# grantjr1842/index-tts

Measured on AMD Instinct MI355X. Metric: synthesised audio seconds per second (IndexTTS-2 infer_v2 hot path), whole job, higher is better.
Workload: dtype f32 (greedy decode + its prefill: exact fp32 MFMA; fp32 accumulate and fp32 activations everywhere) + split-bf16 (fp32 operands as hi+lo bf16, 3 bf16 MFMAs per product) GEMMs, DiT attention and convolutions in s2mel, the latent pass and the vocoder; GPT linear weights STORED as bf16 (rounded once at

## Files before the change

index-tts_amd/csrc/gemm.h:

```cpp
#pragma once
#include "common.h"

namespace idxtts {

enum GemmAct { ACT_NONE = 0, ACT_GELU_NEW = 1, ACT_SILU = 2, ACT_SWIGLU = 3, ACT_MISH = 4, ACT_GATE = 5 ,
               ACT_GELU_ERF = 6 , ACT_RELU = 7  };

struct LinearWeights {
  const float* wp = nullptr;
  const float* bias = nullptr;
  int N = 0, K = 0;
  const void* tiles16 = nullptr;
  const void* planes16 = nullptr;
  bool mf16 = false;
};

static inline size_t linear_packed_floats(int N, int K) { return (size_t)cdiv(N, 32) * cdiv(K, 16) * 512; }

void pack_linear(float* dst, const float* w, int N, int K);

struct GemmArgs {
  const float* x = nullptr; int ldx = 0;
  float* y = nullptr; int ldy = 0;
  const void* x_planes = nullptr;
  void* y_planes = nullptr;
  const float* rope = nullptr; int rope_T = 0, rope_cols = 0;
  const float* res = nullptr; int ldr = 0;
  int M = 0;
  int act = ACT_NONE;
  float out_scale = 1.0f;
  int taps = 1, seq_len = 0, dil = 1, pad_left = 0, pad_mode = 0;
  const int* row_len = nullptr;
  int ksplit = 1;
  int bf16_products = 3;
};

int gemm_tn_forward(const LinearWeights& w, const GemmArgs& a, hipStream_t stream);
int gemm_bf16x3_forward(const LinearWeights& w, const GemmArgs& a, hipStream_t stream);
static inline bool linear_takes_planes(int N, int K) { return N >= 96 && K % 16 == 0; }
size_t linear_tiles_bytes(int N, int K);
void pack_linear_tiles(void* dst, const float* w, int N, int K);
size_t linear_planes_bytes(int N, int K);
void pack_linear_planes(void* dst, const float* w, int N, int K);

enum GemmMode { GEMM_F32 = 0, GEMM_BF16X3 = 1 };
void set_gemm_mode(int mode);
int get_gemm_mode();
void set_acoustic_bf16(int on);
int get_acoustic_bf16();
bool acoustic_bf16_active();
int gemm_forward(const LinearWeights& w, const GemmArgs& a, hipStream_t stream);
bool gemm_uses_planes(const LinearWeights& w, const GemmArgs& a);

int gemm_release_stream_scratch(hipStream_t stream);

}
```

index-tts_amd/csrc/gemm_bf16x3_v2.hip:

```cpp
#include <algorithm>
#include <cstdlib>
#include <cstring>

#include "gemm_common.h"
#include "prof.h"

namespace idxtts {

typedef __bf16 bf16x8 __attribute__((ext_vector_type(8)));
typedef __bf16 bf16x4 __attribute__((ext_vector_type(4)));

size_t linear_planes_bytes(int N, int K) { return (size_t)2 * cdiv(K, 16) * (cdiv(N, 256) * 256) * 16 * sizeof(uint16_t); }

void pack_linear_planes(void* dst, const float* w, int N, int K) {
  uint16_t* o = static_cast<uint16_t*>(dst);
  const int KC = cdiv(K, 16), NP = cdiv(N, 256) * 256;
  std::memset(o, 0, linear_planes_bytes(N, K));
  uint16_t* lo = o + (size_t)KC * NP * 16;
  for (int n = 0; n < N; ++n)
    for (int k = 0; k < K; ++k) {
      const float x = w[(size_t)n * K + k];
      const uint16_t hi = f2bf(x);
      const size_t idx = ((size_t)(k >> 4) * NP + n) * 16 + (k & 15);
      o[idx] = hi;
      lo[idx] = f2bf(x - bf2f(hi));
    }
}

__global__ __launch_bounds__(256) void split_planes_kernel(const float* __restrict__ x, int ldx, int M, int K, __bf16* __restrict__ hi,
                                                           __bf16* __restrict__ lo) {
  const int k = blockIdx.y * 64 + (threadIdx.x & 15) * 4;
#pragma unroll
  for (int i = 0; i < 4; ++i) {
    const int m = blockIdx.x * 64 + (threadIdx.x >> 4) + 16 * i;
    if (m >= M || k >= ((K + 15) & ~15)) continue;
    const f32x4 v = k < K ? *reinterpret_cast<const f32x4*>(x + (size_t)m * ldx + k) : f32x4{0.f, 0.f, 0.f, 0.f};
    bf16x4 h, l;
    split_bf16_x4(v, h, l);
    const size_t o = ((size_t)(k >> 4) * M + m) * 16 + (k & 15);
    *reinterpret_cast<bf16x4*>(hi + o) = h;
    *reinterpret_cast<bf16x4*>(lo + o) = l;
  }
}

#ifdef V2_TIMING
static unsigned long long* g_v2_stamps = nullptr;
extern "C" int idxtts_dbg_v2_stamps(void* buf) { g_v2_stamps = static_cast<unsigned long long*>(buf); return 0; }
#define V2_STAMP(k) do { if (q.stamps && tid == 64) q.stamps[(size_t)blockIdx.x * 8 + (k)] = __builtin_amdgcn_s_memtime(); } while (0)
#define V2_RSTAMP(k) do { if (q.stamps && tid == 64) q.stamps[(size_t)blockIdx.x * 8 + (k)] = __builtin_amdgcn_s_memrealtime(); } while (0)
#else
#define V2_STAMP(k)
#define V2_RSTAMP(k)
#endif

struct GemmV2P {
  GemmKP g;
  const __bf16* a_hi; const __bf16* a_lo;
  const __bf16* b_hi; const __bf16* b_lo;
  int a_rows, npad, nstages;
  int a_bytes, b_bytes;
  int a_plane, b_plane;
  int cs, nbg;
#ifdef V2_TIMING
  unsigned long long* stamps;
#endif
};

struct V2Rsrc { __amdgpu_buffer_rsrc_t a, b; };

#define V2_WAITCNT(vm) __builtin_amdgcn_s_waitcnt(((vm) & 15) | (((vm) >> 4) << 14) | 0x70)

template <bool TAPS, int EPI, int MF, int NP = 3>
__device__ __forceinline__ void gemm_v2_tile(const GemmV2P& q, const int bm, const int bn, const int tid) {
  constexpr int NSTAGE = 3;
  constexpr int WMW = 2, WNW = 2, TN = 2;
  constexpr int BM = 64 * WMW, BN = 32 * TN * WNW;
  static_assert(BM / 32 == WMW * WNW && BN / 32 == WMW * WNW, "one 32-row block of A and of B per wave and plane");
  static_assert(MF == 32 || MF == 16, "MFMA shape");
  static_assert(NP == 3 || (NP == 1 && MF == 16), "one MFMA per product exists in the 16x16x32 loop only");
  constexpr int PLANE = BM * 32;
  constexpr int STAGE_BYTES = 4 * PLANE;
  constexpr int PPW = NP == 1 ? 2 : 4;
  const GemmKP& p = q.g;
  extern __shared__ __attribute__((aligned(1024))) char smv2[];

  const int wave = __builtin_amdgcn_readfirstlane(tid >> 6), lane = tid & 63;
  const int h = lane >> 5, j = lane & 31;
  const int wm = wave >> 1, wn = wave & 1;

  const int lrow = lane >> 1;
  const int dunit = (lane & 1) ^ ((lrow >> 3) & 1);
  const int a_m = bm * BM + 32 * wave + lrow;
  const __amdgpu_buffer_rsrc_t rA = __builtin_amdgcn_make_buffer_rsrc(const_cast<__bf16*>(q.a_hi), 0, q.a_bytes, 0x00020000);
  const __amdgpu_buffer_rsrc_t rB = __builtin_amdgcn_make_buffer_rsrc(const_cast<__bf16*>(q.b_hi), 0, q.b_bytes, 0x00020000);
  const int voffB = (bn * BN + 32 * wave + lrow) * 32 + dunit * 16;
  int voffA = min(a_m, q.a_rows - 1) * 32 + dunit * 16;
  const ConvRow arow = conv_row(p, a_m);
  auto tap_voff = [&](int tap) -> int {
    const int t = conv_src_row(arow.t + tap * p.dil - p.pad_left, arow.n, p.pad_mode);
    return a_m < p.M && t >= 0 ? (arow.base + t) * 32 + dunit * 16 : (int)0x80000000;
  };
  V2_STAMP(0); V2_RSTAMP(4);
  const int ns = q.nstages;
  const int sA = q.a_rows * 32, sB = q.npad * 32;
  const int cpt = TAPS ? (p.kc >> 4) : ns;
  int ist = 0, soA = 0, soB = 0, ich = 0, itap = 0, wslot = 0, rslot = 0;
  if (TAPS) voffA = tap_voff(0);
  char* const lds_w = smv2 + wave * 1024;
  auto issue_piece = [&](int pi) {
    auto dst = (__attribute__((address_space(3))) void*)(lds_w + wslot * STAGE_BYTES + pi * PLANE);
    if (pi == 0) __builtin_amdgcn_raw_ptr_buffer_load_lds(rA, dst, 16, voffA, soA, 0, 0);
    else if (pi == 1) __builtin_amdgcn_raw_ptr_buffer_load_lds(rA, dst, 16, voffA, soA + q.a_plane, 0, 0);
    else if (pi == 2) __builtin_amdgcn_raw_ptr_buffer_load_lds(rB, dst, 16, voffB, soB, 0, 0);
    else __builtin_amdgcn_raw_ptr_buffer_load_lds(rB, dst, 16, voffB, soB + q.b_plane, 0, 0);
  };
  auto issue_a = [&]() { issue_piece(0); if (NP == 3) issue_piece(1); };
  auto issue_b = [&]() { issue_piece(2); if (NP == 3) issue_piece(3); };
  auto advance = [&]() {
    ++ist;
    wslot = wslot + 1 == NSTAGE ? 0 : wslot + 1;
    soB += sB;
    soA += sA;
    if (TAPS) {
      if (++ich == cpt) { ich = 0; soA = 0; ++itap; voffA = tap_voff(itap); }
    }
  };

  if constexpr (MF == 16) {
    const int g = lane >> 4, r16 = lane & 15;
    const int sw = ((g & 1) ^ ((r16 >> 3) & 1)) * 16;
    const int a_off = (wm * 64 + r16) * 32 + sw;
    const int b_off = 2 * PLANE + (wn * 64 + r16) * 32 + sw;
    f32x4 acc[4][4];
#pragma unroll
    for (int a = 0; a < 4; ++a)
#pragma unroll
      for (int b = 0; b < 4; ++b)
#pragma unroll
        for (int r = 0; r < 4; ++r) acc[a][b][r] = 0.0f;
    for (int s = 0; s < NSTAGE; ++s)
      if (s < ns) {
        issue_a(); issue_b();
        advance();
      }

    typedef unsigned u32x4 __attribute__((ext_vector_type(4)));
    auto pair_step = [&](const bool tail, const bool vm_one_behind, const int nreq) {
      if (vm_one_behind) V2_WAITCNT(PPW); else V2_WAITCNT(0);
      __builtin_amdgcn_s_barrier();
      __builtin_amdgcn_sched_barrier(0);
      const int second = rslot + 1 == NSTAGE ? 0 : rslot + 1;
      const char* st = smv2 + ((g >> 1) && !tail ? second : rslot) * STAGE_BYTES;
      rslot = second + 1 == NSTAGE ? 0 : second + 1;
      bf16x8 ah[4], al[4], bh[4], bl[4];
      auto rd_a = [&](int t) {
        ah[t] = *reinterpret_cast<const bf16x8*>(st + a_off + t * 512);
        if (NP == 3) al[t] = *reinterpret_cast<const bf16x8*>(st + PLANE + a_off + t * 512);
      };
      auto rd_b = [&](int t) {
        bh[t] = *reinterpret_cast<const bf16x8*>(st + b_off + t * 512);
        if (NP == 3) bl[t] = *reinterpret_cast<const bf16x8*>(st + PLANE + b_off + t * 512);
      };
      rd_a(0); rd_b(0);
      __builtin_amdgcn_sched_barrier(0);
      rd_a(1);
      __builtin_amdgcn_sched_barrier(0);
      rd_a(2);
      __builtin_amdgcn_sched_barrier(0);
      rd_a(3);
      __builtin_amdgcn_sched_barrier(0);
#pragma unroll
      for (int t = 1; t < 4; ++t) rd_b(t);
      if (tail) {
        const unsigned keep = (g >> 1) ? 0u : 0xffffffffu;
#pragma unroll
        for (int t = 0; t < 4; ++t) {
          ah[t] = (bf16x8)((u32x4)ah[t] & keep); if (NP == 3) al[t] = (bf16x8)((u32x4)al[t] & keep);
          bh[t] = (bf16x8)((u32x4)bh[t] & keep); if (NP == 3) bl[t] = (bf16x8)((u32x4)bl[t] & keep);
        }
      }
      auto prod = [&](int mt, int nt) {
        if (NP == 3) {
          acc[mt][nt] = __builtin_amdgcn_mfma_f32_16x16x32_bf16(al[mt], bh[nt], acc[mt][nt], 0, 0, 0);
          acc[mt][nt] = __builtin_amdgcn_mfma_f32_16x16x32_bf16(ah[mt], bl[nt], acc[mt][nt], 0, 0, 0);
        }
        acc[mt][nt] = __builtin_amdgcn_mfma_f32_16x16x32_bf16(ah[mt], bh[nt], acc[mt][nt], 0, 0, 0);
      };
#define V2_MFMA3(nt) _Pragma("unroll") for (int mt = 0; mt < 4; ++mt) prod(mt, nt);
#define V2_MFMA1(mt, nt) prod(mt, nt); __builtin_amdgcn_sched_barrier(0);

      __builtin_amdgcn_sched_barrier(0);
      V2_MFMA1(0, 0) V2_MFMA1(1, 0) V2_MFMA1(2, 0) V2_MFMA1(3, 0)
      V2_WAITCNT(63);
      __builtin_amdgcn_s_barrier();
      __builtin_amdgcn_sched_barrier(0);
      if (nreq >= 1) issue_a();
      __builtin_amdgcn_sched_barrier(0);
      V2_MFMA3(1)
      __builtin_amdgcn_sched_barrier(0);
      if (nreq >= 1) { issue_b(); advance(); }
      if (nreq >= 2) issue_a();
      __builtin_amdgcn_sched_barrier(0);
      V2_MFMA3(2)
      __builtin_amdgcn_sched_barrier(0);
      if (nreq >= 2) { issue_b(); advance(); }
      __builtin_amdgcn_sched_barrier(0);
      V2_MFMA3(3)
      __builtin_amdgcn_sched_barrier(0);
#undef V2_MFMA1
#undef V2_MFMA3
    };
    V2_STAMP(1);
    int done = 0;
    for (; ist + 2 <= ns && ist > done + 2; done += 2) pair_step(false, true, 2);
    for (; done + 2 <= ns; done += 2) pair_step(false, ist > done + 2, min(ns - ist, 2));
    if (done < ns) pair_step(true, false, 0);
    V2_STAMP(2);
    auto write_pass = [&](int ps, float* lds, int RS) {
#pragma unroll
      for (int nt = 0; nt < 4; ++nt)
#pragma unroll
        for (int e = 0; e < 4; ++e) lds[(4 * g + e) * RS + nt * 16 + r16] = acc[ps][nt][e];
    };
    gemm_epilogue_wave<EPI, TN, 3>(p, write_pass, reinterpret_cast<float*>(smv2), bm * BM + wm * 64, bn * BN + wn * TN * 32, wave, lane);
  } else {
    const int sw = (h ^ ((j >> 3) & 1)) * 16;
    const int a_off = (wm * 64 + j) * 32 + sw;
    const int b_offr = (wn * TN * 32 + j) * 32 + sw;

    f32x16 acc[2][TN];
#pragma unroll
    for (int a = 0; a < 2; ++a)
#pragma unroll
      for (int b = 0; b < TN; ++b)
#pragma unroll
        for (int r = 0; r < 16; ++r) acc[a][b][r] = 0.0f;

    for (int s = 0; s < NSTAGE; ++s)
      if (s < ns) {
#pragma unroll
        for (int pi = 0; pi < PPW; ++pi) issue_piece(pi);
        advance();
      }

    struct Frag { bf16x8 ah[2], al[2], bh[TN], bl[TN]; };
    auto wait_stage = [&](int s) {
      const int rem = ns - 1 - s;
      if (rem >= 1) V2_WAITCNT(PPW);
      else V2_WAITCNT(0);
      __builtin_amdgcn_s_barrier();
      __builtin_amdgcn_sched_barrier(0);
    };
    auto load_frags = [&](Frag& f) {
      const char* st = smv2 + rslot * STAGE_BYTES;
      rslot = rslot + 1 == NSTAGE ? 0 : rslot + 1;
#pragma unroll
      for (int t = 0; t < 2; ++t) {
        f.ah[t] = *reinterpret_cast<const bf16x8*>(st + a_off + t * 1024);
        f.al[t] = *reinterpret_cast<const bf16x8*>(st + PLANE + a_off + t * 1024);
      }
#pragma unroll
      for (int t = 0; t < TN; ++t) {
        f.bh[t] = *reinterpret_cast<const bf16x8*>(st + 2 * PLANE + b_offr + t * 1024);
        f.bl[t] = *reinterpret_cast<const bf16x8*>(st + 3 * PLANE + b_offr + t * 1024);
      }
    };
    auto compute = [&](const Frag& f, const bool more) {
#define V2_MFMA3(mt, nt)                                                                                         \
      acc[mt][nt] = __builtin_amdgcn_mfma_f32_32x32x16_bf16(f.al[mt], f.bh[nt], acc[mt][nt], 0, 0, 0);             \
      acc[mt][nt] = __builtin_amdgcn_mfma_f32_32x32x16_bf16(f.ah[mt], f.bl[nt], acc[mt][nt], 0, 0, 0);             \
      acc[mt][nt] = __builtin_amdgcn_mfma_f32_32x32x16_bf16(f.ah[mt], f.bh[nt], acc[mt][nt], 0, 0, 0);
      V2_MFMA3(0, 0)
      __builtin_amdgcn_sched_barrier(0);
      if (more) issue_piece(0);
      __builtin_amdgcn_sched_barrier(0);
      V2_MFMA3(0, 1)
      __builtin_amdgcn_sched_barrier(0);
      if (more) issue_piece(1);
      __builtin_amdgcn_sched_barrier(0);
      V2_MFMA3(1, 0)
      __builtin_amdgcn_sched_barrier(0);
      if (more) issue_piece(2);
      __builtin_amdgcn_sched_barrier(0);
      V2_MFMA3(1, 1)
      __builtin_amdgcn_sched_barrier(0);
      if (more) { issue_piece(3); advance(); }
      __builtin_amdgcn_sched_barrier(0);
#undef V2_MFMA3
    };

    Frag f0, f1;
    {
      const int rem = ns - 1;
      if (rem >= 2) V2_WAITCNT(2 * PPW);
      else if (rem >= 1) V2_WAITCNT(PPW);
      else V2_WAITCNT(0);
      __builtin_amdgcn_s_barrier();
      __builtin_amdgcn_sched_barrier(0);
    }
    V2_STAMP(1);
    load_frags(f0);
    int i = 0;
    for (; i + NSTAGE + 1 < ns; i += 2) {
      V2_WAITCNT((NSTAGE - 2) * PPW);
      __builtin_amdgcn_s_barrier();
      __builtin_amdgcn_sched_barrier(0);
      load_frags(f1);
      compute(f0, true);
      V2_WAITCNT((NSTAGE - 2) * PPW);
      __builtin_amdgcn_s_barrier();
      __builtin_amdgcn_sched_barrier(0);
      load_frags(f0);
      compute(f1, true);
    }
    for (; i < ns; i += 2) {
      if (i + 1 < ns) { wait_stage(i + 1); load_frags(f1); }
      else V2_WAITCNT(0);
      compute(f0, ist < ns);
      if (i + 1 < ns) {
        if (i + 2 < ns) { wait_stage(i + 2); load_frags(f0); }
        else V2_WAITCNT(0);
        compute(f1, ist < ns);
      }
    }
    V2_STAMP(2);
    auto write_pass = [&](int ps, float* lds, int RS) {
      const int mt = ps >> 1, hh = ps & 1;
#pragma unroll
      for (int nt = 0; nt < TN; ++nt)
#pragma unroll
        for (int qq = 0; qq < 2; ++qq)
#pragma unroll
          for (int e = 0; e < 4; ++e) lds[(8 * qq + 4 * h + e) * RS + nt * 32 + j] = acc[mt][nt][(2 * hh + qq) * 4 + e];
    };
    gemm_epilogue_wave<EPI, TN, 3>(p, write_pass, reinterpret_cast<float*>(smv2), bm * BM + wm * 64, bn * BN + wn * TN * 32, wave, lane);
  }
  V2_STAMP(6);
#ifdef V2_TIMING
  asm volatile("s_waitcnt vmcnt(0)" ::: "memory");
#endif
  V2_STAMP(3); V2_RSTAMP(5);
}

template <bool TAPS, int EPI, int MF, int NP = 3>
__global__ __launch_bounds__(256, 3) void gemm_bf16x3_v2_kernel(const GemmV2P q) {
  int bn, bm;
  if (!gemm_tile_walk(q.g, blockIdx.x, bm, bn, q.cs, q.nbg)) return;
  gemm_v2_tile<TAPS, EPI, MF, NP>(q, bm, bn, threadIdx.x);
}

StreamScratch g_plane_scratch(8);

int gemm_bf16x3_v2_forward(GemmKP p, const LinearWeights& w, const GemmArgs& a, hipStream_t stream, double flops, double bytes) {
  IDX_CHECK(w.K % 16 == 0 && (a.taps <= 1 || (w.K / a.taps) % 16 == 0), "v2 needs K % 16 == 0");
  const int xk = a.taps > 1 ? w.K / a.taps : w.K;
  const size_t plane = (size_t)(xk / 16) * a.M * 16 * sizeof(__bf16);
  void* scratch = nullptr;
  if (!a.x_planes && g_plane_scratch.acquire(stream, 2 * plane, &scratch)) return 1;
  const __bf16* hi = static_cast<const __bf16*>(a.x_planes ? a.x_planes : scratch);
  const __bf16* lo = hi + plane / sizeof(__bf16);
  if (!a.x_planes) {
    static const int cat_split = prof_register("split_planes_kernel");
    ProfScope prof(cat_split, stream, 0.0, 8.0 * a.M * (double)xk);
    hipLaunchKernelGGL(split_planes_kernel, dim3(cdiv(a.M, 64), cdiv(xk, 64)), dim3(256), 0, stream, a.x, a.ldx, a.M, xk, const_cast<__bf16*>(hi), const_cast<__bf16*>(lo));
    IDX_LAUNCH_CHECK();
  }
  GemmV2P q;
  q.g = p;
  if (a.y_planes) {
    const int n_out = (a.act == ACT_SWIGLU || a.act == ACT_GATE) ? w.N / 2 : w.N;
    IDX_CHECK(n_out % 16 == 0 && (a.ldy & 3) == 0, "output planes need N_out % 16 == 0");
    q.g.y_hi = static_cast<__bf16*>(a.y_planes);
    q.g.y_lo = q.g.y_hi + plane_elems(a.M, n_out);
  }
  if (a.rope) {
    IDX_CHECK(a.rope_T > 0 && a.rope_cols % 64 == 0 && a.act == ACT_NONE && (a.ldy & 3) == 0, "fused rotary arguments");
    q.g.rope = a.rope; q.g.rope_T = a.rope_T; q.g.rope_cols = a.rope_cols;
  }
  const int BMh = 128, BNh = 128;
  q.g.mtiles = cdiv(a.M, BMh);
  q.g.mt8 = cdiv(q.g.mtiles, 8);
  q.g.nblocks = cdiv(w.N, BNh);
  q.a_hi = hi; q.a_lo = lo; q.a_rows = a.M;
  q.npad = cdiv(w.N, 256) * 256;
  q.b_hi = static_cast<const __bf16*>(w.planes16);
  q.b_lo = q.b_hi + (size_t)(w.K / 16) * q.npad * 16;
  q.nstages = w.K / 16;
#ifdef V2_TIMING
  q.stamps = g_v2_stamps;
#endif
  const size_t b_plane = (size_t)(w.K / 16) * q.npad * 32;
  IDX_CHECK(2 * plane < (1ull << 31) && 2 * b_plane < (1ull << 31), "operand planes beyond the 2 GiB a buffer offset addresses");
  q.a_plane = (int)plane; q.a_bytes = (int)(2 * plane);
  q.b_plane = (int)b_plane; q.b_bytes = (int)(2 * b_plane);
  q.cs = 1;
  static const double cs_bytes = [] { const char* e = getenv("IDXTTS_GEMM_CS_BYTES"); return e ? atof(e) : 3.2e6; }();
  if (!q.g.n_fast && (double)w.N * w.K * 4.0 <= 8.0 * cs_bytes && a.M > w.N) q.g.n_fast = 1;
  if (q.g.n_fast) {
    while (q.cs < 8 && (double)w.N * w.K * 4.0 / q.cs > cs_bytes && q.g.nblocks >= 2 * q.cs) q.cs *= 2;
  }
  q.nbg = cdiv(q.g.nblocks, q.cs);
  const int64_t grid = q.g.n_fast ? (int64_t)8 * q.nbg * cdiv(q.g.mtiles, 8 / q.cs) : (int64_t)8 * q.g.nblocks * q.g.mt8;
  IDX_CHECK(grid < (1ll << 31), "grid size");
  static const int cat = prof_register("gemm_bf16x3_v2_kernel");
  ProfScope prof(cat, stream, flops, bytes);
  const int lds = 3 * (4 * 128 * 32);
  const bool paired = a.act == ACT_SWIGLU || a.act == ACT_GATE;
  IDX_CHECK(!(a.rope && (a.res || paired)), "the rotary epilogue takes no residual and no paired activation");
  IDX_CHECK(!a.row_len || a.seq_len >= 16, "row masks need seq_len >= 16");
  const int epi = a.rope ? EPI_ROPE : paired ? EPI_PAIRED : a.act != ACT_NONE ? EPI_ACT : EPI_PLAIN;
  typedef void (*KernelFn)(const GemmV2P);
#define V2_ROW(T, F, P) gemm_bf16x3_v2_kernel<T, EPI_PLAIN, F, P>, gemm_bf16x3_v2_kernel<T, EPI_ROPE, F, P>, gemm_bf16x3_v2_kernel<T, EPI_PAIRED, F, P>, gemm_bf16x3_v2_kernel<T, EPI_ACT, F, P>
  static const KernelFn kernels[3][2][4] = {{{V2_ROW(false, 32, 3)}, {V2_ROW(true, 32, 3)}}, {{V2_ROW(false, 16, 3)}, {V2_ROW(true, 16, 3)}},
                                            {{V2_ROW(false, 16, 1)}, {V2_ROW(true, 16, 1)}}};
  static DynLdsLimit lds_limit;
  IDX_HIP(lds_limit.set(lds, V2_ROW(false, 32, 3), V2_ROW(true, 32, 3), V2_ROW(false, 16, 3), V2_ROW(true, 16, 3), V2_ROW(false, 16, 1), V2_ROW(true, 16, 1)));
  IDX_CHECK(a.bf16_products == 3 || (a.bf16_products == 1 && w.mf16), "one MFMA per product needs weights of the 16x16x32 loop");
  int mf16 = w.mf16 ? 1 : 0;
#ifdef V2_EXP_SHAPE
  if (const char* e = getenv("IDXTTS_EXP_V2_SHAPE")) mf16 = atoi(e) == 16;
#endif
  const KernelFn kernel = kernels[a.bf16_products == 1 ? 2 : mf16][a.taps > 1 ? 1 : 0][epi];
#undef V2_ROW
  hipLaunchKernelGGL(kernel, dim3((unsigned)grid), dim3(256), lds, stream, q);
  IDX_LAUNCH_CHECK();
  return 0;
}

}
```

index-tts_amd/csrc/model_util.h:

```cpp
#pragma once
#include <map>
#include <string>
#include <vector>

#include "ctx.h"
#include "gemm.h"

namespace idxtts {

int need(std::map<std::string, HostTensor>& t, const std::string& key, std::vector<int64_t> shape, HostTensor** out);
int up(DeviceArena& arena, const std::vector<float>& v, const float** out);
int tensor_from(std::map<std::string, HostTensor>& t, DeviceArena& arena, const std::string& key, std::vector<int64_t> shape, const float** out);
int vec_from(std::map<std::string, HostTensor>& t, DeviceArena& arena, const std::string& key, int n, const float** out);
int ln_from(std::map<std::string, HostTensor>& t, DeviceArena& arena, const std::string& prefix, int n, const float** g, const float** b);

enum Wp16Policy {
  WP16_ALWAYS,
  WP16_DMA_SHAPES,
  WP16_ALWAYS_MF16,
  WP16_NONE,
};
enum WeightLayout { W_NK , W_KN  };
struct LinearOpts {
  Wp16Policy wp16;
  WeightLayout layout = W_NK;
  int Kpad = 0;
  bool split_bf16_below_256_rows = false;
};
int make_linear(DeviceArena& arena, const float* w, const float* bias, int N, int K, const LinearOpts& o, LinearWeights* out);
int linear_from(std::map<std::string, HostTensor>& t, DeviceArena& arena, const std::string& prefix, int N, int K, bool bias, Wp16Policy wp16,
                LinearWeights* out, std::vector<int64_t> wshape = {});

struct Carver {
  char* base; size_t off = 0;
  explicit Carver(void* b) : base(static_cast<char*>(b)) {}
  template <typename T> T* take(size_t n) {
    off = (off + 255) & ~(size_t)255;
    T* p = base ? reinterpret_cast<T*>(base + off) : nullptr;
    off += n * sizeof(T);
    return p;
  }
};

int lin(const LinearWeights& w, const float* x, int ldx, float* y, int ldy, int M, hipStream_t st, int act = ACT_NONE,
        const float* res = nullptr, int ldr = 0);
int lin_exact(const LinearWeights& w, const float* x, int ldx, float* y, int ldy, int M, hipStream_t st, int act = ACT_NONE,
              const float* res = nullptr, int ldr = 0);
int layer_norm(const float* x, float* y, const float* g, const float* b, int M, int d, hipStream_t st);

}
```

index-tts_amd/csrc/model_util.hip:

```cpp
#include "model_util.h"

#include <cstring>

#include "norm.h"

namespace idxtts {

int need(std::map<std::string, HostTensor>& t, const std::string& key, std::vector<int64_t> shape, HostTensor** out) {
  auto it = t.find(key);
  if (it == t.end()) IDX_FAIL("missing tensor '" + key + "'");
  if (it->second.shape != shape) {
    std::string s = "tensor '" + key + "' has shape [";
    for (auto d : it->second.shape) s += std::to_string(d) + ",";
    s += "] expected [";
    for (auto d : shape) s += std::to_string(d) + ",";
    IDX_FAIL(s + "]");
  }
  *out = &it->second;
  return 0;
}

int up(DeviceArena& arena, const std::vector<float>& v, const float** out) {
  float* d = nullptr;
  if (arena.upload(v.data(), v.size(), &d)) return 1;
  *out = d;
  return 0;
}

int tensor_from(std::map<std::string, HostTensor>& t, DeviceArena& arena, const std::string& key, std::vector<int64_t> shape, const float** out) {
  HostTensor* h = nullptr;
  if (need(t, key, shape, &h)) return 1;
  return up(arena, h->data, out);
}

int vec_from(std::map<std::string, HostTensor>& t, DeviceArena& arena, const std::string& key, int n, const float** out) {
  return tensor_from(t, arena, key, {n}, out);
}

int ln_from(std::map<std::string, HostTensor>& t, DeviceArena& arena, const std::string& prefix, int n, const float** g, const float** b) {
  return vec_from(t, arena, prefix + ".weight", n, g) || vec_from(t, arena, prefix + ".bias", n, b);
}

int make_linear(DeviceArena& arena, const float* w, const float* bias, int N, int K, const LinearOpts& o, LinearWeights* out) {
  const int Kpad = o.Kpad ? o.Kpad : K;
  IDX_CHECK(Kpad >= K, "Kpad < K");
  std::vector<float> rows;
  if (o.layout == W_KN || Kpad != K) {
    rows.assign((size_t)N * Kpad, 0.0f);
    for (int n = 0; n < N; ++n)
      for (int k = 0; k < K; ++k) rows[(size_t)n * Kpad + k] = o.layout == W_KN ? w[(size_t)k * N + n] : w[(size_t)n * K + k];
    w = rows.data();
  }
  std::vector<float> packed(linear_packed_floats(N, Kpad));
  pack_linear(packed.data(), w, N, Kpad);
  if (up(arena, packed, &out->wp)) return 1;
  out->N = N; out->K = Kpad;
  out->mf16 = o.wp16 == WP16_ALWAYS_MF16;
  auto pack16 = [&](size_t bytes, void (*pack)(void*, const float*, int, int), const void** dst) {
    std::vector<float> p16((bytes + 3) / 4);
    pack(p16.data(), w, N, Kpad);
    const float* d16 = nullptr;
    if (up(arena, p16, &d16)) return 1;
    *dst = d16;
    return 0;
  };
  const bool planes = o.wp16 != WP16_NONE && linear_takes_planes(N, Kpad);
  const bool tiles = o.wp16 != WP16_NONE && (o.split_bf16_below_256_rows || (o.wp16 != WP16_DMA_SHAPES && !planes));
  if (planes && pack16(linear_planes_bytes(N, Kpad), pack_linear_planes, &out->planes16)) return 1;
  if (tiles && pack16(linear_tiles_bytes(N, Kpad), pack_linear_tiles, &out->tiles16)) return 1;
  if (bias && up(arena, std::vector<float>(bias, bias + N), &out->bias)) return 1;
  return 0;
}

int linear_from(std::map<std::string, HostTensor>& t, DeviceArena& arena, const std::string& prefix, int N, int K, bool bias, Wp16Policy wp16,
                LinearWeights* out, std::vector<int64_t> wshape) {
  HostTensor *w = nullptr, *b = nullptr;
  if (wshape.empty()) wshape = {N, K};
  if (need(t, prefix + ".weight", wshape, &w)) return 1;
  if (bias && need(t, prefix + ".bias", {N}, &b)) return 1;
  return make_linear(arena, w->data.data(), b ? b->data.data() : nullptr, N, K, {wp16, W_NK, (K + 3) & ~3}, out);
}

static GemmArgs lin_args(const float* x, int ldx, float* y, int ldy, int M, int act, const float* res, int ldr) {
  GemmArgs g;
  g.x = x; g.ldx = ldx; g.y = y; g.ldy = ldy; g.M = M; g.act = act; g.res = res; g.ldr = ldr;
  return g;
}

int lin(const LinearWeights& w, const float* x, int ldx, float* y, int ldy, int M, hipStream_t st, int act, const float* res, int ldr) {
  const GemmArgs g = lin_args(x, ldx, y, ldy, M, act, res, ldr);
  if (act == ACT_GELU_ERF || act == ACT_RELU) return gemm_tn_forward(w, g, st);
  return gemm_forward(w, g, st);
}

int lin_exact(const LinearWeights& w, const float* x, int ldx, float* y, int ldy, int M, hipStream_t st, int act, const float* res, int ldr) {
  return gemm_tn_forward(w, lin_args(x, ldx, y, ldy, M, act, res, ldr), st);
}

int layer_norm(const float* x, float* y, const float* g, const float* b, int M, int d, hipStream_t st) {
  RowsNormArgs n;
  n.x_in = x; n.ld_in = d; n.y = y; n.ld_y = d; n.M = M; n.d = d; n.mode = NORM_LN; n.eps = 1e-5f; n.g1 = g; n.b1 = b;
  return rows_norm_forward(n, st);
}

}
```

index-tts_amd/csrc/s2mel.hip:

```cpp
#include <cmath>
#include <cstring>

#include <map>
#include <mutex>
#include <utility>

#include "model_util.h"
#include "s2mel.h"
#include "s2mel_buffers.h"

namespace idxtts {

S2MelModel::S2MelModel(const idxtts_s2mel_config& c) : cfg(c) {}

bool S2MelModel::accepts(const std::string& name) const {
  static const char* prefixes[] = {"cfm.estimator.", "length_regulator.", "gpt_layer.", "semantic_codec.", "rope_cache"};
  for (const char* p : prefixes)
    if (name.rfind(p, 0) == 0) return true;
  return false;
}

namespace {

std::vector<float> col_slice(const std::vector<float>& w, int N, int K, int k0, int k1) {
  std::vector<float> o((size_t)N * (k1 - k0));
  for (int n = 0; n < N; ++n) std::memcpy(&o[(size_t)n * (k1 - k0)], &w[(size_t)n * K + k0], (k1 - k0) * sizeof(float));
  return o;
}

std::vector<float> pair_pack(const float* a, const float* b, int H, int K) {
  std::vector<float> o((size_t)2 * H * K);
  for (int blk = 0; blk < H / 32; ++blk) {
    std::memcpy(&o[(size_t)(blk * 64) * K], a + (size_t)blk * 32 * K, (size_t)32 * K * sizeof(float));
    std::memcpy(&o[(size_t)(blk * 64 + 32) * K], b + (size_t)blk * 32 * K, (size_t)32 * K * sizeof(float));
  }
  return o;
}

std::vector<float> conv_to_rows(const std::vector<float>& w, int Cout, int Cin, int k) {
  std::vector<float> o((size_t)Cout * Cin * k);
  for (int co = 0; co < Cout; ++co)
    for (int ci = 0; ci < Cin; ++ci)
      for (int kk = 0; kk < k; ++kk) o[((size_t)co * k + kk) * Cin + ci] = w[((size_t)co * Cin + ci) * k + kk];
  return o;
}

}

int S2MelModel::finalize(std::map<std::string, HostTensor>& t, DeviceArena& arena) {
  const int D = cfg.hidden_dim, C = cfg.in_channels, Wh = cfg.wn_hidden, depth = cfg.depth;
  IDX_CHECK(D == cfg.num_heads * 64, "head_dim must be 64");
  IDX_CHECK(Wh == D, "the reference's FinalLayer requires wavenet.hidden_dim == DiT.hidden_dim");
  IDX_CHECK((D & 31) == 0 && (Wh & 31) == 0 && (cfg.lr_channels & 31) == 0, "channel counts must be multiples of 32");
  {
    const int nh = (int)(2 * (4 * D) / 3);
    ffn = (nh % 256 == 0) ? nh : nh + 256 - (nh % 256);
  }
  const std::string e = "cfm.estimator";
  auto lin_from = [&](const std::string& key, int N, int K, bool bias, LinearWeights* out) { return linear_from(t, arena, key, N, K, bias, WP16_ALWAYS_MF16, out); };
  auto mk_lin = [&](const float* w, const float* bias, int N, int K, LinearWeights* out) { return make_linear(arena, w, bias, N, K, {WP16_ALWAYS_MF16}, out); };
  blocks.resize(depth);
  std::vector<float> mod_w, mod_b;
  auto append_mod = [&](const std::string& name) -> int {
    HostTensor *w = nullptr, *b = nullptr;
    if (need(t, name + ".project_layer.weight", {2 * D, D}, &w) || need(t, name + ".project_layer.bias", {2 * D}, &b)) return 1;
    mod_w.insert(mod_w.end(), w->data.begin(), w->data.end());
    mod_b.insert(mod_b.end(), b->data.begin(), b->data.end());
    return 0;
  };
  for (int i = 0; i < depth; ++i) {
    DiTBlock& B = blocks[i];
    const std::string p = e + ".transformer.layers." + std::to_string(i);
    if (lin_from(p + ".attention.wqkv", 3 * D, D, false, &B.wqkv)) return 1;
    if (lin_from(p + ".attention.wo", D, D, false, &B.wo)) return 1;
    HostTensor *w1 = nullptr, *w3 = nullptr;
    if (need(t, p + ".feed_forward.w1.weight", {ffn, D}, &w1) || need(t, p + ".feed_forward.w3.weight", {ffn, D}, &w3)) return 1;
    if (mk_lin(pair_pack(w1->data.data(), w3->data.data(), ffn, D).data(), nullptr, 2 * ffn, D, &B.w13)) return 1;
    if (lin_from(p + ".feed_forward.w2", D, ffn, false, &B.w2)) return 1;
    HostTensor *g = nullptr;
    if (need(t, p + ".attention_norm.norm.weight", {D}, &g) || up(arena, g->data, &B.attn_g)) return 1;
    if (need(t, p + ".ffn_norm.norm.weight", {D}, &g) || up(arena, g->data, &B.ffn_g)) return 1;
    if (append_mod(p + ".attention_norm") || append_mod(p + ".ffn_norm")) return 1;
    if (i > depth / 2) {
      HostTensor *sw = nullptr, *sb = nullptr;
      if (need(t, p + ".skip_in_linear.weight", {D, 2 * D}, &sw) || need(t, p + ".skip_in_linear.bias", {D}, &sb)) return 1;
      if (mk_lin(col_slice(sw->data, D, 2 * D, 0, D).data(), sb->data.data(), D, D, &B.skip_a)) return 1;
      if (mk_lin(col_slice(sw->data, D, 2 * D, D, 2 * D).data(), nullptr, D, D, &B.skip_b)) return 1;
    }
  }
  {
    HostTensor* g = nullptr;
    if (need(t, e + ".transformer.norm.norm.weight", {D}, &g) || up(arena, g->data, &final_g)) return 1;
    if (append_mod(e + ".transformer.norm")) return 1;
    if (mk_lin(mod_w.data(), mod_b.data(), (2 * depth + 1) * 2 * D, D, &mod_all)) return 1;
  }
  const int Win = 2 * C + D + cfg.style_dim;
  if (lin_from(e + ".cond_projection", D, cfg.content_dim, true, &cond_proj)) return 1;
  if (lin_from(e + ".cond_x_merge_linear", D, Win, true, &merge)) return 1;
  if (lin_from(e + ".t_embedder.mlp.0", D, 256, true, &temb0) || lin_from(e + ".t_embedder.mlp.2", D, D, true, &temb2)) return 1;
  if (lin_from(e + ".t_embedder2.mlp.0", Wh, 256, true, &t2emb0) || lin_from(e + ".t_embedder2.mlp.2", Wh, Wh, true, &t2emb2)) return 1;
  {
    HostTensor *sw = nullptr, *sb = nullptr;
    if (need(t, e + ".skip_linear.weight", {D, D + C}, &sw) || need(t, e + ".skip_linear.bias", {D}, &sb)) return 1;
    if (mk_lin(col_slice(sw->data, D, D + C, 0, D).data(), sb->data.data(), D, D, &skiplin_a)) return 1;
    if (mk_lin(col_slice(sw->data, D, D + C, D, D + C).data(), nullptr, D, C, &skiplin_b)) return 1;
  }
  if (lin_from(e + ".conv1", Wh, D, true, &conv1)) return 1;
  if (lin_from(e + ".res_projection", Wh, D, true, &res_proj)) return 1;
  if (lin_from(e + ".final_layer.linear", Wh, Wh, true, &final_lin)) return 1;
  if (lin_from(e + ".final_layer.adaLN_modulation.1", 2 * Wh, Wh, true, &final_mod)) return 1;
  {
    HostTensor *w = nullptr, *b = nullptr;
    if (need(t, e + ".conv2.weight", {C, Wh, 1}, &w) || need(t, e + ".conv2.bias", {C}, &b)) return 1;
    if (mk_lin(w->data.data(), b->data.data(), C, Wh, &conv2)) return 1;
  }
  const int L = cfg.wn_layers, k = cfg.wn_kernel;
  wn.resize(L);
  {
    HostTensor *cw = nullptr, *cb = nullptr;
    if (need(t, e + ".wavenet.cond_layer.conv.conv.weight", {2 * Wh * L, Wh, 1}, &cw) ||
        need(t, e + ".wavenet.cond_layer.conv.conv.bias", {2 * Wh * L}, &cb)) return 1;
    std::vector<float> cw_perm, cb_perm;
    for (int l = 0; l < L; ++l) {
      WNLayer& W = wn[l];
      const std::string p = e + ".wavenet.in_layers." + std::to_string(l) + ".conv.conv";
      HostTensor *iw = nullptr, *ib = nullptr;
      if (need(t, p + ".weight", {2 * Wh, Wh, k}, &iw) || need(t, p + ".bias", {2 * Wh}, &ib)) return 1;
      const std::vector<float> rows = conv_to_rows(iw->data, 2 * Wh, Wh, k);
      if (mk_lin(pair_pack(rows.data(), rows.data() + (size_t)Wh * k * Wh, Wh, k * Wh).data(), nullptr, 2 * Wh, k * Wh, &W.in_gate)) return 1;
      const float* cwl = cw->data.data() + (size_t)l * 2 * Wh * Wh;
      const std::vector<float> cwp = pair_pack(cwl, cwl + (size_t)Wh * Wh, Wh, Wh);
      cw_perm.insert(cw_perm.end(), cwp.begin(), cwp.end());
      std::vector<float> bsum(2 * Wh);
      for (int c = 0; c < 2 * Wh; ++c) bsum[c] = cb->data[(size_t)l * 2 * Wh + c] + ib->data[c];
      const std::vector<float> bp = pair_pack(bsum.data(), bsum.data() + Wh, Wh, 1);
      cb_perm.insert(cb_perm.end(), bp.begin(), bp.end());
      const std::string r = e + ".wavenet.res_skip_layers." + std::to_string(l) + ".conv.conv";
      const int rc = l < L - 1 ? 2 * Wh : Wh;
      HostTensor *rw = nullptr, *rb = nullptr;
      if (need(t, r + ".weight", {rc, Wh, 1}, &rw) || need(t, r + ".bias", {rc}, &rb)) return 1;
      if (l < L - 1) {
        std::vector<float> w_res(rw->data.begin(), rw->data.begin() + (size_t)Wh * Wh), b_res(rb->data.begin(), rb->data.begin() + Wh);
        std::vector<float> w_skip(rw->data.begin() + (size_t)Wh * Wh, rw->data.end()), b_skip(rb->data.begin() + Wh, rb->data.end());
        if (mk_lin(w_res.data(), b_res.data(), Wh, Wh, &W.res) || mk_lin(w_skip.data(), b_skip.data(), Wh, Wh, &W.skip)) return 1;
      } else {
        W.has_res = false;
        if (mk_lin(rw->data.data(), rb->data.data(), Wh, Wh, &W.skip)) return 1;
      }
    }
    if (mk_lin(cw_perm.data(), cb_perm.data(), 2 * Wh * L, Wh, &wn_cond)) return 1;
  }
  const int LC = cfg.lr_channels;
  if (lin_from("length_regulator.content_in_proj", LC, cfg.lr_in_channels, true, &lr_in)) return 1;
  lr_conv.resize(cfg.lr_num_convs);
  lr_gn_g.resize(cfg.lr_num_convs);
  lr_gn_b.resize(cfg.lr_num_convs);
  for (int n = 0; n < cfg.lr_num_convs; ++n) {
    HostTensor *w = nullptr, *b = nullptr, *g = nullptr, *bb = nullptr;
    const std::string p = "length_regulator.model." + std::to_string(3 * n);
    if (need(t, p + ".weight", {LC, LC, 3}, &w) || need(t, p + ".bias", {LC}, &b)) return 1;
    if (mk_lin(conv_to_rows(w->data, LC, LC, 3).data(), b->data.data(), LC, 3 * LC, &lr_conv[n])) return 1;
    const std::string q = "length_regulator.model." + std::to_string(3 * n + 1);
    if (need(t, q + ".weight", {LC}, &g) || need(t, q + ".bias", {LC}, &bb)) return 1;
    if (up(arena, g->data, &lr_gn_g[n]) || up(arena, bb->data, &lr_gn_b[n])) return 1;
  }
  {
    HostTensor *w = nullptr, *b = nullptr;
    const std::string p = "length_regulator.model." + std::to_string(3 * cfg.lr_num_convs);
    if (need(t, p + ".weight", {LC, LC, 1}, &w) || need(t, p + ".bias", {LC}, &b)) return 1;
    if (mk_lin(w->data.data(), b->data.data(), LC, LC, &lr_out)) return 1;
  }
  {
    const int dims[4] = {cfg.gpt_dim, cfg.gpt_layer_dims[0], cfg.gpt_layer_dims[1], cfg.gpt_layer_dims[2]};
    for (int n = 0; n < 3; ++n)
      if (lin_from("gpt_layer." + std::to_string(n), dims[n + 1], dims[n], true, &gl[n])) return 1;
    IDX_CHECK(dims[3] == cfg.codec_hidden && cfg.codec_hidden == cfg.lr_in_channels, "gpt_layer / codec / length-regulator widths");
  }
  {
    HostTensor *cb = nullptr, *ow = nullptr, *ob = nullptr;
    const std::string q = "semantic_codec.quantizer.quantizers.0";
    if (need(t, q + ".codebook.weight", {cfg.codebook_size, cfg.codebook_dim}, &cb) ||
        need(t, q + ".out_project.weight", {cfg.codec_hidden, cfg.codebook_dim, 1}, &ow) ||
        need(t, q + ".out_project.bias", {cfg.codec_hidden}, &ob)) return 1;
    std::vector<float> table((size_t)cfg.codebook_size * cfg.codec_hidden);
    for (int v = 0; v < cfg.codebook_size; ++v)
      for (int h = 0; h < cfg.codec_hidden; ++h) {
        float acc = 0.0f;
        for (int c = 0; c < cfg.codebook_dim; ++c) acc = std::fmaf(cb->data[(size_t)v * cfg.codebook_dim + c], ow->data[(size_t)h * cfg.codebook_dim + c], acc);
        table[(size_t)v * cfg.codec_hidden + h] = acc + ob->data[h];
      }
    if (up(arena, table, &vq_table)) return 1;
  }
  {
    auto it = t.find("rope_cache");
    if (it == t.end()) IDX_FAIL("missing tensor 'rope_cache' ([T][32][2] cos/sin table, precompute_freqs_cis)");
    IDX_CHECK(it->second.shape.size() == 3 && it->second.shape[1] == 32 && it->second.shape[2] == 2, "rope_cache must be [T][32][2]");
    rope_len = (int)it->second.shape[0];
    if (up(arena, it->second.data, &rope)) return 1;
  }
  return 0;
}

size_t S2MelModel::cfm_workspace_bytes(int B, int T, int n_steps) const { return carve_cfm(cfg, ffn, nullptr, B, T, n_steps).bytes; }

struct Src { const float* f; const void* p; Src(const float* rows, const void* planes = nullptr) : f(planes ? nullptr : rows), p(planes) {} };
struct Dst { float* f; void* p; Dst(float* rows, void* planes = nullptr) : f(rows), p(planes) {} };

static GemmArgs gemm_args(Src x, int ldx, Dst y, int ldy, int M, int act = ACT_NONE, const float* res = nullptr, int ldr = 0) {
  GemmArgs a;
  a.x = x.f; a.x_planes = x.p; a.ldx = ldx; a.y = y.f; a.y_planes = y.p; a.ldy = ldy; a.M = M; a.act = act; a.res = res; a.ldr = ldr;
  return a;
}
static int gemm(const LinearWeights& w, Src x, int ldx, Dst y, int ldy, int M, hipStream_t st, int act = ACT_NONE,
                const float* res = nullptr, int ldr = 0) {
  return gemm_forward(w, gemm_args(x, ldx, y, ldy, M, act, res, ldr), st);
}

struct RowSet {
  const CfmBuffers* w = nullptr;
  int nseq = 0, seq = 0, rows = 0;
  const int* lens = nullptr;
  bool planes = false;
  bool planes_wn = false;

  Src hn_in() const { return in(w->hn, w->hn_p, planes); }                  Dst hn_out() const { return instead(w->hn, w->hn_p, planes); }
  Src att_in() const { return in(w->att, w->att_p, planes); }               Dst att_out() const { return instead(w->att, w->att_p, planes); }
  Src ff_in() const { return in(w->ff, w->ff_p, planes); }                  Dst ff_out() const { return instead(w->ff, w->ff_p, planes); }
  Src acts_in() const { return in(w->wn_acts, w->acts_p, planes); }         Dst acts_out() const { return instead(w->wn_acts, w->acts_p, planes); }
  Src skip_in(int i) const { return in(w->skips[i], w->skips_p[i], planes); }   Dst skip_out(int i) const { return beside(w->skips[i], w->skips_p[i], planes); }
  Src xres_in() const { return in(w->xres, w->xres_p, planes_wn); }         Dst xres_out() const { return beside(w->xres, w->xres_p, planes_wn); }
  Src wnx_in() const { return in(w->wn_x, w->wnx_p, planes_wn); }           Dst wnx_out() const { return beside(w->wn_x, w->wnx_p, planes_wn); }
  Src h_in(const float* h) const { return in(h, w->h_p, planes); }          Dst h_out(float* h, bool reread) const { return beside(h, w->h_p, planes && reread); }

 private:
  static Src in(const float* f, const void* p, bool on) { return on ? Src(f, p) : Src(f); }
  static Dst instead(float* f, void* p, bool on) { return on ? Dst(nullptr, p) : Dst(f); }
  static Dst beside(float* f, void* p, bool on) { return on ? Dst(f, p) : Dst(f); }
};

static RowSet row_set(const S2MelModel& m, const CfmBuffers& w, int nseq, int seq, const int* lens, const RowSet* within) {
  RowSet r;
  r.w = &w; r.nseq = nseq; r.seq = seq; r.rows = nseq * seq; r.lens = lens;
  const DiTBlock& b0 = m.blocks[0];
  const WNLayer& wn0 = m.wn[0];
  GemmArgs pr;
  pr.M = r.rows;
  r.planes = within ? within->planes : gemm_uses_planes(b0.wqkv, pr);
  for (const LinearWeights* lw : {&b0.wo, &b0.w13, &b0.w2, &m.skiplin_a, &m.final_lin, &wn0.skip}) r.planes = r.planes && gemm_uses_planes(*lw, pr);
  r.planes_wn = r.planes && (!within || within->planes_wn);
  for (const LinearWeights* lw : {&m.skiplin_b, &m.conv1, &m.res_proj, &wn0.res}) r.planes_wn = r.planes_wn && gemm_uses_planes(*lw, pr);
  pr.taps = m.cfg.wn_kernel; pr.seq_len = seq;
  r.planes_wn = r.planes_wn && gemm_uses_planes(wn0.in_gate, pr);
  return r;
}

static int ada_norm(const S2MelModel& m, const float* x, const float* g, const float* mod, const RowSet& r, hipStream_t st) {
  const int D = m.cfg.hidden_dim;
  const Dst hn = r.hn_out();
  RowsNormArgs n;
  n.x_in = x; n.ld_in = D; n.y = hn.f; n.y_planes = hn.p; n.ld_y = D; n.M = r.rows; n.d = D;
  n.mode = NORM_ADA_RMS; n.eps = m.cfg.norm_eps; n.g1 = g;
  n.mod_a = mod; n.mod_b = mod + D; n.ld_mod = 0; n.rows_per_batch = 0;
  return rows_norm_forward(n, st);
}

static int attention(const S2MelModel& m, const RowSet& all, bool qkv_planes, int q0, int Sq, Dst o, hipStream_t st) {
  const int D = m.cfg.hidden_dim, T = all.seq;
  const float* qkv = all.w->qkv;
  if (qkv_planes) {
    AttnPlanesArgs ap;
    ap.planes = qkv; ap.Mrows = all.rows; ap.ncols = 3 * D; ap.q_col = 0; ap.k_col = D; ap.v_col = 2 * D; ap.T = T; ap.q_row0 = q0; ap.Sq = Sq;
    ap.B = all.nseq; ap.H = m.cfg.num_heads; ap.kend = all.lens; ap.scale = 0.125f;
    ap.o = o.f; ap.o_planes = o.p; ap.o_bs = (long)Sq * D; ap.o_ts = D;
    ap.split_bf16 = acoustic_bf16_active() ? 2 : 1;
    return flash_attn_planes_forward(ap, st);
  }
  AttnArgs a;
  a.q = qkv + (size_t)q0 * 3 * D; a.k = qkv + D; a.v = qkv + 2 * D; a.o = o.f; a.o_planes = o.p;
  a.q_bs = a.k_bs = a.v_bs = (long)T * 3 * D; a.o_bs = (long)Sq * D; a.q_ts = a.k_ts = a.v_ts = 3 * D; a.o_ts = D;
  a.B = all.nseq; a.H = m.cfg.num_heads; a.Sq = Sq; a.Sk = T; a.causal = 0; a.kend = all.lens; a.scale = 0.125f;
  a.split_bf16 = get_gemm_mode() == GEMM_BF16X3 ? (acoustic_bf16_active() ? 2 : 1) : 0;
  return flash_attn_forward(a, st);
}

static int dit_block(S2MelModel& m, int i, const float* mods, const float* h, const RowSet& all, const RowSet& post, float* res, Dst out,
                     hipEvent_t lag_event, hipStream_t st) {
  const auto& c = m.cfg;
  const CfmBuffers& w = *all.w;
  const DiTBlock& B = m.blocks[i];
  const int D = c.hidden_dim, T = all.seq, q0 = T - post.seq;
  if (ada_norm(m, h, B.attn_g, mods + (size_t)(2 * i) * 2 * D, all, st)) return 1;
  bool qkv_planes = false;
  {
    GemmArgs g = gemm_args(all.hn_in(), D, w.qkv, 3 * D, all.rows);
    const bool fuse_rope = gemm_uses_planes(B.wqkv, g);
    qkv_planes = fuse_rope && D == 64 * c.num_heads;
    if (fuse_rope) { g.rope = m.rope; g.rope_T = T; g.rope_cols = 2 * D; }
    if (qkv_planes) { g.y = nullptr; g.y_planes = w.qkv; }
    if (gemm_forward(B.wqkv, g, st)) return 1;
    if (!fuse_rope && rotary_qk(w.qkv, all.rows, c.num_heads, T, m.rope, st)) return 1;
  }
  if (attention(m, all, qkv_planes, q0, post.seq, post.att_out(), st)) return 1;
  if (lag_event) IDX_HIP(hipEventRecord(lag_event, st));
  if (res != h && gather_tail_rows(res, D, h, D, D, all.nseq, T, q0, st)) return 1;
  if (gemm(B.wo, post.att_in(), D, w.hmid, D, post.rows, st, ACT_NONE, res, D)) return 1;
  if (ada_norm(m, w.hmid, B.ffn_g, mods + (size_t)(2 * i + 1) * 2 * D, post, st)) return 1;
  if (gemm(B.w13, post.hn_in(), D, post.ff_out(), m.ffn, post.rows, st, ACT_SWIGLU)) return 1;
  return gemm(B.w2, post.ff_in(), m.ffn, out, D, post.rows, st, ACT_NONE, w.hmid, D);
}

static int dit_eval(S2MelModel& m, CfmBuffers& w, int N2, int T, int step, hipStream_t st, hipEvent_t lag_event) {
  const auto& c = m.cfg;
  const int D = c.hidden_dim, C = c.in_channels, Wh = c.wn_hidden, depth = c.depth, half = depth / 2;
  const int Win = 2 * C + D + c.style_dim;
  const float* mods = w.mods + (size_t)step * (2 * depth + 1) * 2 * D;
  const int t0 = w.tail_t0;
  const RowSet all = row_set(m, w, N2, T, w.lens2, nullptr);
  const RowSet tail = t0 > 0 ? row_set(m, w, N2, T - t0, w.lens2t, &all) : all;
  if (lag_event && depth < 2) IDX_HIP(hipEventRecord(lag_event, st));
  if (gemm(m.merge, w.x_in, Win, w.ha, D, all.rows, st)) return 1;
  float* h = w.ha;
  int pushed = 0;
  for (int i = 0; i < depth; ++i) {
    if (i > half) {
      DiTBlock& B = m.blocks[i];
      --pushed;
      if (gemm(B.skip_a, all.h_in(h), D, w.hmid, D, all.rows, st)) return 1;
      float* dst = (h == w.ha) ? w.hb : w.ha;
      if (gemm(B.skip_b, all.skip_in(pushed), D, dst, D, all.rows, st, ACT_NONE, w.hmid, D)) return 1;
      h = dst;
    }
    const Dst out = i < half ? all.skip_out(pushed) : all.h_out((h == w.ha) ? w.hb : w.ha, i + 1 < depth && i + 1 > half);
    const bool cut = i == depth - 1 && t0 > 0;
    if (dit_block(m, i, mods, h, all, cut ? tail : all, cut ? w.xres : h, out, i == 0 && !cut ? lag_event : nullptr, st)) return 1;
    if (i < half) ++pushed;
    h = out.f;
  }
  const int Mt = tail.rows, Tt = tail.seq;
  const float* xin_t = w.x_in;
  int ld_xin = Win;
  if (t0 > 0) {
    if (gather_tail_rows(w.qkv, C, w.x_in, Win, C, N2, T, t0, st)) return 1;
    xin_t = w.qkv; ld_xin = C;
  }
  if (ada_norm(m, h, m.final_g, mods + (size_t)(2 * depth) * 2 * D, tail, st)) return 1;
  if (gemm(m.skiplin_a, tail.hn_in(), D, w.hmid, D, Mt, st)) return 1;
  if (gemm(m.skiplin_b, xin_t, ld_xin, tail.xres_out(), D, Mt, st, ACT_NONE, w.hmid, D)) return 1;
  if (gemm(m.conv1, tail.xres_in(), D, tail.wnx_out(), Wh, Mt, st)) return 1;
  const int L = c.wn_layers, k = c.wn_kernel;
  for (int l = 0; l < L; ++l) {
    WNLayer& W = m.wn[l];
    int dil = 1;
    for (int q = 0; q < l; ++q) dil *= c.wn_dilation_rate;
    LinearWeights in = W.in_gate;
    in.bias = w.wnb + ((size_t)step * L + l) * 2 * Wh;
    GemmArgs g = gemm_args(tail.wnx_in(), Wh, tail.acts_out(), Wh, Mt, ACT_GATE);
    g.taps = k; g.seq_len = Tt; g.dil = dil; g.pad_left = (k - 1) / 2 * dil; g.pad_mode = 1; g.row_len = tail.lens;
    if (gemm_forward(in, g, st)) return 1;
    if (W.has_res) {
      GemmArgs r = gemm_args(tail.acts_in(), Wh, tail.wnx_out(), Wh, Mt, ACT_NONE, w.wn_x, Wh);
      r.seq_len = Tt; r.row_len = tail.lens;
      if (gemm_forward(W.res, r, st)) return 1;
    }
    GemmArgs sk = gemm_args(tail.acts_in(), Wh, w.wn_out, Wh, Mt);
    if (l > 0) { sk.res = w.wn_out; sk.ldr = Wh; }
    if (l == L - 1) { sk.seq_len = Tt; sk.row_len = tail.lens; }
    if (gemm_forward(W.skip, sk, st)) return 1;
  }
  if (gemm(m.res_proj, tail.xres_in(), D, w.hmid, Wh, Mt, st, ACT_NONE, w.wn_out, Wh)) return 1;
  {
    const Dst hn = tail.hn_out();
    RowsNormArgs n;
    n.x_in = w.hmid; n.ld_in = Wh; n.y = hn.f; n.y_planes = hn.p; n.ld_y = Wh; n.M = Mt; n.d = Wh; n.mode = NORM_MOD_LN; n.eps = 1e-6f;
    n.mod_a = w.fmod + (size_t)step * 2 * Wh; n.mod_b = n.mod_a + Wh; n.ld_mod = 0; n.rows_per_batch = 0;
    if (rows_norm_forward(n, st)) return 1;
  }
  if (gemm(m.final_lin, tail.hn_in(), Wh, w.att, Wh, Mt, st)) return 1;
  return gemm(m.conv2, w.att, Wh, w.vout, C, Mt, st);
}

struct HalfStreams { hipStream_t side = nullptr; hipEvent_t fork = nullptr, lag = nullptr, join = nullptr; };
static std::map<std::pair<int, hipStream_t>, HalfStreams> g_half_streams;
static std::mutex g_half_mu;
static int g_s2mel_overlap = 0;
void set_s2mel_overlap(int on) { g_s2mel_overlap = on ? 1 : 0; }
int get_s2mel_overlap() { return g_s2mel_overlap; }

static int half_streams_for(hipStream_t st, HalfStreams* out) {
  int dev = 0;
  IDX_HIP(hipGetDevice(&dev));
  std::lock_guard<std::mutex> lk(g_half_mu);
  HalfStreams& hs = g_half_streams[std::make_pair(dev, st)];
  if (!hs.side) {
    int prio = 0;
    if (st) IDX_HIP(hipStreamGetPriority(st, &prio));
    IDX_HIP(hipStreamCreateWithPriority(&hs.side, hipStreamNonBlocking, prio));
    IDX_HIP(hipEventCreateWithFlags(&hs.fork, hipEventDisableTiming));
    IDX_HIP(hipEventCreateWithFlags(&hs.lag, hipEventDisableTiming));
    IDX_HIP(hipEventCreateWithFlags(&hs.join, hipEventDisableTiming));
  }
  *out = hs;
  return 0;
}

int s2mel_release_stream(hipStream_t st) {
  int dev = 0;
  IDX_HIP(hipGetDevice(&dev));
  HalfStreams hs;
  {
    std::lock_guard<std::mutex> lk(g_half_mu);
    auto it = g_half_streams.find(std::make_pair(dev, st));
    if (it == g_half_streams.end()) return 0;
    hs = it->second;
    g_half_streams.erase(it);
  }
  if (hs.side) { (void)hipStreamSynchronize(hs.side); (void)hipStreamDestroy(hs.side); }
  if (hs.fork) (void)hipEventDestroy(hs.fork);
  if (hs.lag) (void)hipEventDestroy(hs.lag);
  if (hs.join) (void)hipEventDestroy(hs.join);
  return 0;
}

static bool halves_on_two_streams(hipStream_t st) {
  hipStreamCaptureStatus cap = hipStreamCaptureStatusNone;
  (void)hipStreamIsCapturing(st, &cap);
  return g_s2mel_overlap && !prof_enabled() && cap == hipStreamCaptureStatusNone;
}

static int dit_eval_halves(S2MelModel& m, CfmBuffers& w, int B, int T, int step, bool two_streams, hipStream_t st) {
  if (!two_streams) return dit_eval(m, w, 2 * B, T, step, st, nullptr);
  CfmBuffers v0 = half_view(m.cfg, m.ffn, w, 0, B, T);
  CfmBuffers v1 = half_view(m.cfg, m.ffn, w, 1, B, T);
  HalfStreams hs;
  if (half_streams_for(st, &hs)) return 1;
  IDX_HIP(hipEventRecord(hs.fork, st));
  IDX_HIP(hipStreamWaitEvent(hs.side, hs.fork, 0));
  if (dit_eval(m, v0, B, T, step, st, hs.lag)) return 1;
  IDX_HIP(hipStreamWaitEvent(hs.side, hs.lag, 0));
  if (dit_eval(m, v1, B, T, step, hs.side, nullptr)) return 1;
  IDX_HIP(hipEventRecord(hs.join, hs.side));
  IDX_HIP(hipStreamWaitEvent(st, hs.join, 0));
  return 0;
}

int S2MelModel::cfm(const float* mu, const int* x_lens_host, const float* prompt, const int* prompt_lens_host, int Tp_max,
                    const float* style, const float* z, const float* t_emb, const float* dt_host, int n_steps, float cfg_rate,
                    float* out, int B, int T, void* ws, size_t ws_bytes, hipStream_t st) {
  IDX_CHECK(mu && x_lens_host && prompt && prompt_lens_host && style && z && t_emb && dt_host && out, "null pointer");
  IDX_CHECK(B > 0 && T > 0 && n_steps > 0 && Tp_max > 0, "shape");
  IDX_CHECK(cfg_rate > 0.0f, "the stacked-CFG path needs inference_cfg_rate > 0 (reference default 0.7)");
  IDX_CHECK(T <= rope_len, "sequence longer than the rope cache");
  IDX_CHECK(ws && ws_bytes >= cfm_workspace_bytes(B, T, n_steps), "workspace too small");
  CfmBuffers w = carve_cfm(cfg, ffn, ws, B, T, n_steps);
  if (cfm_solve(w, mu, x_lens_host, prompt, prompt_lens_host, Tp_max, style, z, t_emb, dt_host, n_steps, cfg_rate, B, T, st)) return 1;
  IDX_HIP(hipMemcpyAsync(out, w.xstate, (size_t)B * cfg.in_channels * T * sizeof(float), hipMemcpyDeviceToDevice, st));
  return 0;
}

static int upload_lens(const S2MelModel& m, CfmBuffers& w, const int* x_lens_host, const int* prompt_lens_host, int Tp_max, int B, int T,
                       bool solver, hipStream_t st) {
  const auto& c = m.cfg;
  std::vector<int> lens2(2 * B), plen(B), lens2t(2 * B);
  for (int b = 0; b < B; ++b) {
    const int pmax = std::min(Tp_max, solver ? x_lens_host[b] : T);
    IDX_CHECK(x_lens_host[b] > 0 && x_lens_host[b] <= T && prompt_lens_host[b] >= 0 && prompt_lens_host[b] <= pmax, "lengths");
    lens2[b] = lens2[B + b] = x_lens_host[b];
    plen[b] = prompt_lens_host[b];
  }
  IDX_HIP(hipMemcpyAsync(w.lens2, lens2.data(), 2 * B * sizeof(int), hipMemcpyHostToDevice, st));
  if (solver) {
    int halo = 0, dil = 1, pmin = plen[0];
    for (int l = 0; l < c.wn_layers; ++l) { halo += (c.wn_kernel - 1) / 2 * dil; dil *= c.wn_dilation_rate; }
    for (int b = 0; b < B; ++b) pmin = std::min(pmin, plen[b]);
    w.tail_t0 = pmin - halo >= 64 ? pmin - halo : 0;
    for (int i = 0; i < 2 * B; ++i) lens2t[i] = lens2[i] - w.tail_t0;
    IDX_HIP(hipMemcpyAsync(w.lens2t, lens2t.data(), 2 * B * sizeof(int), hipMemcpyHostToDevice, st));
  }
  IDX_HIP(hipMemcpyAsync(w.plen, plen.data(), B * sizeof(int), hipMemcpyHostToDevice, st));
  IDX_HIP(hipStreamSynchronize(st));
  return 0;
}

static int step_constants(const S2MelModel& m, const CfmBuffers& w, const float* t_emb, int n_steps, hipStream_t st) {
  const int D = m.cfg.hidden_dim, Wh = m.cfg.wn_hidden;
  if (gemm(m.temb0, t_emb, 256, w.tmp_steps, D, n_steps, st, ACT_SILU) || gemm(m.temb2, w.tmp_steps, D, w.t1, D, n_steps, st)) return 1;
  if (gemm(m.mod_all, w.t1, D, w.mods, (2 * m.cfg.depth + 1) * 2 * D, n_steps, st)) return 1;
  if (silu_rows(w.t1s, w.t1, (size_t)n_steps * D, st) || gemm(m.final_mod, w.t1s, Wh, w.fmod, 2 * Wh, n_steps, st)) return 1;
  if (gemm(m.t2emb0, t_emb, 256, w.tmp_steps, Wh, n_steps, st, ACT_SILU) || gemm(m.t2emb2, w.tmp_steps, Wh, w.t2, Wh, n_steps, st)) return 1;
  return gemm(m.wn_cond, w.t2, Wh, w.wnb, m.cfg.wn_layers * 2 * Wh, n_steps, st);
}

static CfmPackArgs pack_args(const S2MelModel& m, const CfmBuffers& w, const float* prompt, const float* style, int B, int T, int Tp_max) {
  const auto& c = m.cfg;
  CfmPackArgs pk;
  pk.x_in = w.x_in; pk.ld = 2 * c.in_channels + c.hidden_dim + c.style_dim; pk.x = w.xstate; pk.prompt = prompt; pk.prompt_len = w.plen;
  pk.cond = w.condp; pk.cond_null = m.cond_proj.bias; pk.style = style;
  pk.B = B; pk.T = T; pk.C = c.in_channels; pk.D = c.hidden_dim; pk.S = c.style_dim; pk.Tp_max = Tp_max;
  return pk;
}

int S2MelModel::cfm_solve(CfmBuffers& w, const float* mu, const int* x_lens_host, const float* prompt, const int* prompt_lens_host,
                          int Tp_max, const float* style, const float* z, const float* t_emb, const float* dt_host, int n_steps,
                          float cfg_rate, int B, int T, hipStream_t st) {
  const int D = cfg.hidden_dim, C = cfg.in_channels;
  if (upload_lens(*this, w, x_lens_host, prompt_lens_host, Tp_max, B, T, true, st)) return 1;
  if (step_constants(*this, w, t_emb, n_steps, st)) return 1;
  if (gemm(cond_proj, mu, cfg.content_dim, w.condp, D, B * T, st)) return 1;
  if (cfm_init_state(w.xstate, z, w.plen, B, C, T, st)) return 1;
  const bool two_streams = halves_on_two_streams(st);
  for (int s = 0; s < n_steps; ++s) {
    CfmPackArgs pk = pack_args(*this, w, prompt, style, B, T, Tp_max);
    pk.x_only = s > 0;
    if (cfm_pack(pk, st)) return 1;
    if (dit_eval_halves(*this, w, B, T, s, two_streams, st)) return 1;
    CfmEulerArgs eu;
    eu.x = w.xstate; eu.v = w.vout; eu.v_null = two_streams ? w.vout + (size_t)B * T * C : nullptr; eu.ldv = C; eu.prompt_len = w.plen; eu.B = B; eu.T = T; eu.C = C; eu.dt = dt_host[s]; eu.cfg_rate = cfg_rate;
    eu.v_t0 = w.tail_t0; eu.v_T = T - w.tail_t0;
    if (cfm_euler(eu, st)) return 1;
  }
  return 0;
}

struct CfmRowsBuffers { float *mu, *prompt; const float **pcond, **ref_mel; int* gen_len; size_t bytes; };

static CfmRowsBuffers carve_cfm_rows(const S2MelModel& m, void* ws, size_t base, int B, int T, int Tp_max) {
  const auto& c = m.cfg;
  CfmRowsBuffers b;
  Carver k(ws ? static_cast<char*>(ws) + base : nullptr);
  b.mu = k.take<float>((size_t)B * T * c.content_dim);
  b.prompt = k.take<float>((size_t)B * c.in_channels * Tp_max);
  b.pcond = k.take<const float*>(B);
  b.ref_mel = k.take<const float*>(B);
  b.gen_len = k.take<int>(B);
  b.bytes = base + ((k.off + 255) & ~(size_t)255);
  return b;
}

size_t S2MelModel::cfm_rows_workspace_bytes(int B, int T, int Tp_max, int n_steps) const {
  return carve_cfm_rows(*this, nullptr, cfm_workspace_bytes(B, T, n_steps), B, T, Tp_max).bytes;
}

int S2MelModel::cfm_rows(const float* gen_cond, const int* target_lens_host, int Tg_max, const float* const* prompt_cond_host,
                         const float* const* ref_mel_host, const int* prompt_lens_host, const float* style, const float* z,
                         const float* t_emb, const float* dt_host, int n_steps, float cfg_rate, float* out, int B, int T, void* ws,
                         size_t ws_bytes, hipStream_t st) {
  IDX_CHECK(gen_cond && target_lens_host && prompt_cond_host && ref_mel_host && prompt_lens_host && style && z && t_emb && dt_host && out,
            "null pointer");
  IDX_CHECK(B > 0 && T > 0 && Tg_max > 0 && n_steps > 0, "shape");
  IDX_CHECK(cfg_rate > 0.0f, "the stacked-CFG path needs inference_cfg_rate > 0 (reference default 0.7)");
  IDX_CHECK(T <= rope_len, "sequence longer than the rope cache");
  IDX_CHECK(cfg.content_dim % 4 == 0 && ((uintptr_t)gen_cond & 15) == 0, "gen_cond must be 16-byte aligned (content_dim % 4 == 0)");
  std::vector<int> xl(B), tg(B);
  int Tp_max = 0, T_need = 0;
  for (int b = 0; b < B; ++b) {
    const int Tp = prompt_lens_host[b], Tg = target_lens_host[b];
    IDX_CHECK(Tp > 0 && Tg > 0 && Tg <= Tg_max, "prompt_lens / target_lens out of range");
    IDX_CHECK(prompt_cond_host[b] && ref_mel_host[b], "null prompt table entry");
    IDX_CHECK(((uintptr_t)prompt_cond_host[b] & 15) == 0, "prompt_condition rows must be 16-byte aligned");
    xl[b] = Tp + Tg;
    tg[b] = Tg;
    Tp_max = std::max(Tp_max, Tp);
    T_need = std::max(T_need, Tp + Tg);
  }
  IDX_CHECK(T == T_need, "T must be max_b(prompt_lens[b] + target_lens[b])");
  IDX_CHECK(ws && ws_bytes >= cfm_rows_workspace_bytes(B, T, Tp_max, n_steps), "workspace too small");
  CfmBuffers w = carve_cfm(cfg, ffn, ws, B, T, n_steps);
  CfmRowsBuffers r = carve_cfm_rows(*this, ws, w.bytes, B, T, Tp_max);
  IDX_HIP(hipMemcpyAsync(r.pcond, prompt_cond_host, B * sizeof(float*), hipMemcpyHostToDevice, st));
  IDX_HIP(hipMemcpyAsync(r.ref_mel, ref_mel_host, B * sizeof(float*), hipMemcpyHostToDevice, st));
  IDX_HIP(hipMemcpyAsync(r.gen_len, tg.data(), B * sizeof(int), hipMemcpyHostToDevice, st));
  IDX_HIP(hipMemcpyAsync(w.plen, prompt_lens_host, B * sizeof(int), hipMemcpyHostToDevice, st));
  CfmRowsPackArgs pk;
  pk.mu = r.mu; pk.prompt = r.prompt; pk.pcond = r.pcond; pk.ref_mel = r.ref_mel; pk.gen = gen_cond; pk.prompt_len = w.plen;
  pk.gen_len = r.gen_len; pk.B = B; pk.T = T; pk.Dc = cfg.content_dim; pk.C = cfg.in_channels; pk.Tp_max = Tp_max; pk.Tg_max = Tg_max;
  if (cfm_rows_pack(pk, st)) return 1;
  if (cfm_solve(w, r.mu, xl.data(), r.prompt, prompt_lens_host, Tp_max, style, z, t_emb, dt_host, n_steps, cfg_rate, B, T, st)) return 1;
  return cfm_rows_emit(out, w.xstate, w.plen, r.gen_len, B, cfg.in_channels, T, Tg_max, st);
}

int S2MelModel::estimator(const float* x, const float* prompt, const int* prompt_lens_host, int Tp_max, const int* x_lens_host,
                          const float* t_emb, const float* style, const float* mu, float* out_tm, int B, int T, void* ws, size_t ws_bytes,
                          hipStream_t st) {
  IDX_CHECK(x && prompt && prompt_lens_host && x_lens_host && t_emb && style && mu && out_tm, "null pointer");
  IDX_CHECK(B > 0 && T > 0 && Tp_max > 0 && T <= rope_len, "shape");
  IDX_CHECK(ws && ws_bytes >= cfm_workspace_bytes(B, T, 1), "workspace too small");
  const int C = cfg.in_channels;
  CfmBuffers w = carve_cfm(cfg, ffn, ws, B, T, 1);
  if (upload_lens(*this, w, x_lens_host, prompt_lens_host, Tp_max, B, T, false, st)) return 1;
  if (step_constants(*this, w, t_emb, 1, st)) return 1;
  if (gemm(cond_proj, mu, cfg.content_dim, w.condp, cfg.hidden_dim, B * T, st)) return 1;
  IDX_HIP(hipMemcpyAsync(w.xstate, x, (size_t)B * C * T * sizeof(float), hipMemcpyDeviceToDevice, st));
  if (cfm_pack(pack_args(*this, w, prompt, style, B, T, Tp_max), st)) return 1;
  {
    CfmBuffers v0 = half_view(cfg, ffn, w, 0, B, T);
    if (dit_eval(*this, v0, B, T, 0, st, nullptr)) return 1;
  }
  IDX_HIP(hipMemcpyAsync(out_tm, w.vout, (size_t)B * T * C * sizeof(float), hipMemcpyDeviceToDevice, st));
  return 0;
}


static CondBuffers carve_cond(const S2MelModel& m, void* ws, int B, int M, int Tg) {
  const auto& c = m.cfg;
  CondBuffers b;
  Carver k(ws);
  const size_t rows = (size_t)B * std::max(M, Tg);
  const int wide = std::max(std::max(c.codec_hidden, c.lr_channels), std::max(c.gpt_layer_dims[0], c.gpt_layer_dims[1]));
  b.a = k.take<float>(rows * wide);
  b.b = k.take<float>(rows * wide);
  b.s = k.take<float>(rows * wide);
  b.stats = k.take<float>(2 * B);
  b.idx_code = k.take<int>((size_t)B * M);
  b.idx_row = k.take<int>((size_t)B * M);
  b.idx_interp = k.take<int>((size_t)B * Tg);
  b.tlen = k.take<int>(B);
  b.bytes = (k.off + 255) & ~(size_t)255;
  return b;
}

size_t S2MelModel::cond_workspace_bytes(int B, int M, int Tg) const { return carve_cond(*this, nullptr, B, M, Tg).bytes; }

static void nearest_rows(int* idx, int row0, int mb, int tb) {
  const float scale = (float)mb / (float)tb;
  for (int j = 0; j < tb; ++j) idx[j] = row0 + std::min((int)std::floor((float)j * scale), mb - 1);
}

int S2MelModel::prepare_cond(const float* latent, const long long* codes, const int* code_lens_host, const int* target_lens_host,
                             int B, int M, int Tg, float* cond_out, void* ws, size_t ws_bytes, hipStream_t st) {
  IDX_CHECK(latent && codes && code_lens_host && target_lens_host && cond_out, "null pointer");
  IDX_CHECK(B > 0 && M > 0 && Tg > 0, "shape");
  IDX_CHECK(ws && ws_bytes >= cond_workspace_bytes(B, M, Tg), "workspace too small");
  const int Hc = cfg.codec_hidden;
  CondBuffers w = carve_cond(*this, ws, B, M, Tg);
  std::vector<long long> hc((size_t)B * M);
  IDX_HIP(hipMemcpyAsync(hc.data(), codes, hc.size() * sizeof(long long), hipMemcpyDeviceToHost, st));
  IDX_HIP(hipStreamSynchronize(st));
  std::vector<int> ic((size_t)B * M), ir((size_t)B * M), ii((size_t)B * Tg, -1), tl(B);
  for (int b = 0; b < B; ++b) {
    const int mb = code_lens_host[b], tb = target_lens_host[b];
    IDX_CHECK(mb > 0 && mb <= M && tb > 0 && tb <= Tg, "code_lens / target_lens out of range");
    tl[b] = tb;
    for (int i = 0; i < M; ++i) {
      const long long cde = hc[(size_t)b * M + i];
      IDX_CHECK(i >= mb || (cde >= 0 && cde < cfg.codebook_size), "semantic code out of the codebook");
      ic[(size_t)b * M + i] = i < mb ? (int)cde : -1;
      ir[(size_t)b * M + i] = i < mb ? b * M + i : -1;
    }
    nearest_rows(&ii[(size_t)b * Tg], b * M, mb, tb);
  }
  IDX_HIP(hipMemcpyAsync(w.idx_code, ic.data(), ic.size() * sizeof(int), hipMemcpyHostToDevice, st));
  IDX_HIP(hipMemcpyAsync(w.idx_row, ir.data(), ir.size() * sizeof(int), hipMemcpyHostToDevice, st));
  IDX_HIP(hipMemcpyAsync(w.idx_interp, ii.data(), ii.size() * sizeof(int), hipMemcpyHostToDevice, st));
  IDX_HIP(hipMemcpyAsync(w.tlen, tl.data(), B * sizeof(int), hipMemcpyHostToDevice, st));
  IDX_HIP(hipStreamSynchronize(st));
  const int rowsM = B * M;
  if (gemm(gl[0], latent, cfg.gpt_dim, w.a, gl[0].N, rowsM, st) || gemm(gl[1], w.a, gl[0].N, w.b, gl[1].N, rowsM, st) ||
      gemm(gl[2], w.b, gl[1].N, w.a, Hc, rowsM, st)) return 1;
  GatherArgs ga;
  ga.out = w.s; ga.ld_out = Hc; ga.d = Hc;
  ga.table[0] = vq_table; ga.idx[0] = w.idx_code;
  ga.table[1] = w.a; ga.idx[1] = w.idx_row;
  if (gather_sum_rows(ga, rowsM, st)) return 1;
  return regulate_rows(w.s, w, B, M, Tg, cond_out, st);
}

int S2MelModel::regulate_rows(const float* s_rows, const CondBuffers& w, int B, int M, int Tg, float* cond_out, hipStream_t st) {
  const int Hc = cfg.codec_hidden, LC = cfg.lr_channels;
  const int rowsM = B * M, rowsT = B * Tg;
  if (gemm(lr_in, s_rows, Hc, w.a, LC, rowsM, st)) return 1;
  GatherArgs gi;
  gi.out = w.b; gi.ld_out = LC; gi.d = LC; gi.table[0] = w.a; gi.idx[0] = w.idx_interp;
  if (gather_sum_rows(gi, rowsT, st)) return 1;
  float* cur = w.b;
  float* other = w.a;
  for (int n = 0; n < cfg.lr_num_convs; ++n) {
    GemmArgs g;
    g.x = cur; g.ldx = LC; g.y = other; g.ldy = LC; g.M = rowsT; g.taps = 3; g.seq_len = Tg; g.dil = 1; g.pad_left = 1; g.pad_mode = 0;
    if (gemm_forward(lr_conv[n], g, st)) return 1;
    if (groupnorm1_mish(cur, other, lr_gn_g[n], lr_gn_b[n], w.tlen, B, Tg, LC, 1e-5f, w.stats, st)) return 1;
  }
  GemmArgs o;
  o.x = cur; o.ldx = LC; o.y = cond_out; o.ldy = LC; o.M = rowsT; o.seq_len = Tg; o.row_len = w.tlen;
  return gemm_forward(lr_out, o, st);
}

int S2MelModel::regulate(const float* S, const int* in_lens_host, const int* target_lens_host, int B, int M, int Tg, float* cond_out,
                         void* ws, size_t ws_bytes, hipStream_t st) {
  IDX_CHECK(S && in_lens_host && target_lens_host && cond_out, "null pointer");
  IDX_CHECK(B > 0 && M > 0 && Tg > 0, "shape");
  IDX_CHECK(ws && ws_bytes >= cond_workspace_bytes(B, M, Tg), "workspace too small");
  CondBuffers w = carve_cond(*this, ws, B, M, Tg);
  std::vector<int> ii((size_t)B * Tg, -1), tl(B);
  for (int b = 0; b < B; ++b) {
    const int mb = in_lens_host[b], tb = target_lens_host[b];
    IDX_CHECK(mb > 0 && mb <= M && tb > 0 && tb <= Tg, "in_lens / target_lens out of range");
    tl[b] = tb;
    nearest_rows(&ii[(size_t)b * Tg], b * M, mb, tb);
  }
  IDX_HIP(hipMemcpyAsync(w.idx_interp, ii.data(), ii.size() * sizeof(int), hipMemcpyHostToDevice, st));
  IDX_HIP(hipMemcpyAsync(w.tlen, tl.data(), B * sizeof(int), hipMemcpyHostToDevice, st));
  IDX_HIP(hipStreamSynchronize(st));
  return regulate_rows(S, w, B, M, Tg, cond_out, st);
}

}
```

index-tts_amd/csrc/s2mel_buffers.h:

```cpp
#pragma once
#include <algorithm>
#include <vector>

#include "../../include/idxtts.h"
#include "model_util.h"

namespace idxtts {

struct CfmBuffers {
  float *x_in, *ha, *hb, *hmid, *hn, *qkv, *att, *ff, *xres, *wn_x, *wn_acts, *wn_out, *vout, *condp, *xstate;
  void *hn_p, *att_p, *ff_p, *acts_p;
  void *h_p, *wnx_p, *xres_p;
  std::vector<void*> skips_p;
  std::vector<float*> skips;
  float *t1, *t1s, *mods, *fmod, *t2, *wnb, *tmp_steps;
  int *lens2, *plen, *lens2t;
  int tail_t0 = 0;
  size_t bytes;
};

enum CfmKind {
  CFM_ROWS,
  CFM_PLANES,
  CFM_STEPS,
  CFM_INTS,
};
constexpr bool CFM_HALVED = true, CFM_SHARED = false;

inline size_t cfm_block_elems(int B, int T, int n_steps, CfmKind kind, size_t cols) {
  return cols * (kind == CFM_STEPS ? (size_t)n_steps : kind == CFM_INTS ? (size_t)B : (size_t)B * T);
}

template <typename F> void cfm_buffer_table(CfmBuffers& b, const idxtts_s2mel_config& c, int ffn, F&& f) {
  const int D = c.hidden_dim, C = c.in_channels, Wh = c.wn_hidden;
  const CfmKind R = CFM_ROWS, P = CFM_PLANES, S = CFM_STEPS;
  const bool H = CFM_HALVED;
  f(b.x_in, 2 * C + D + c.style_dim, R, H); f(b.ha, D, R, H); f(b.hb, D, R, H); f(b.hmid, D, R, H); f(b.hn, D, R, H);
  f(b.qkv, 3 * D, R, H); f(b.att, D, R, H); f(b.ff, ffn, R, H); f(b.xres, D, R, H);
  f(b.hn_p, std::max(D, Wh), P, H); f(b.att_p, D, P, H); f(b.ff_p, ffn, P, H); f(b.acts_p, Wh, P, H);
  f(b.h_p, D, P, H); f(b.wnx_p, Wh, P, H); f(b.xres_p, D, P, H);
  f(b.wn_x, Wh, R, H); f(b.wn_acts, Wh, R, H); f(b.wn_out, Wh, R, H); f(b.vout, C, R, H);
  f(b.condp, D, R, CFM_SHARED);
  f(b.xstate, C, R, CFM_SHARED);
  for (float*& s : b.skips) f(s, D, R, H);
  for (void*& s : b.skips_p) f(s, D, P, H);
  f(b.t1, D, S, CFM_SHARED); f(b.t1s, D, S, CFM_SHARED); f(b.tmp_steps, std::max(D, Wh), S, CFM_SHARED);
  f(b.mods, (2 * c.depth + 1) * 2 * D, S, CFM_SHARED); f(b.fmod, 2 * Wh, S, CFM_SHARED); f(b.t2, Wh, S, CFM_SHARED);
  f(b.wnb, c.wn_layers * 2 * Wh, S, CFM_SHARED);
  f(b.lens2, 1, CFM_INTS, H); f(b.plen, 1, CFM_INTS, CFM_SHARED); f(b.lens2t, 1, CFM_INTS, H);
}

template <typename T> inline void cfm_take(T*& p, Carver& k, size_t n) { p = k.take<T>(n); }
inline void cfm_take(void*& p, Carver& k, size_t n) { p = k.take<float>(n); }
template <typename T> inline void cfm_advance(T*& p, size_t n) { p += n; }
inline void cfm_advance(void*& p, size_t n) { p = static_cast<float*>(p) + n; }

inline CfmBuffers carve_cfm(const idxtts_s2mel_config& c, int ffn, void* ws, int B, int T, int n_steps) {
  CfmBuffers b;
  b.skips.resize(c.depth / 2);
  b.skips_p.resize(c.depth / 2);
  Carver k(ws);
  cfm_buffer_table(b, c, ffn, [&](auto*& p, size_t cols, CfmKind kind, bool halved) {
    cfm_take(p, k, (halved ? 2 : 1) * cfm_block_elems(B, T, n_steps, kind, cols));
  });
  b.bytes = (k.off + 255) & ~(size_t)255;
  return b;
}

inline CfmBuffers half_view(const idxtts_s2mel_config& c, int ffn, const CfmBuffers& w, int h, int B, int T) {
  CfmBuffers v = w;
  cfm_buffer_table(v, c, ffn, [&](auto*& p, size_t cols, CfmKind kind, bool halved) {
    if (halved) cfm_advance(p, h * cfm_block_elems(B, T, 0, kind, cols));
  });
  return v;
}

}
```

index-tts_amd/csrc/s2mel_ops.h:

```cpp
#pragma once
#include "common.h"

namespace idxtts {

int rotary_qk(float* qkv, int M, int H, int seq_len, const float* rope , hipStream_t st);
int silu_rows(float* y, const float* x, size_t n, hipStream_t st);

struct CfmPackArgs {
  float* x_in; int ld;
  const float* x;
  const float* prompt;
  const int* prompt_len;
  const float* cond;
  const float* cond_null;
  const float* style;
  int B, T, C, D, S, Tp_max;
  int x_only = 0;
};
int cfm_pack(const CfmPackArgs& a, hipStream_t st);

struct CfmEulerArgs {
  float* x;
  const float* v; int ldv;
  const float* v_null = nullptr;
  const int* prompt_len;
  int B, T, C;
  float dt, cfg_rate;
  int v_t0 = 0, v_T = 0;
};
int cfm_euler(const CfmEulerArgs& a, hipStream_t st);

struct CfmRowsPackArgs {
  float* mu;
  float* prompt;
  const float* const* pcond;
  const float* const* ref_mel;
  const float* gen;
  const int* prompt_len;
  const int* gen_len;
  int B, T, Dc, C, Tp_max, Tg_max;
};
int cfm_rows_pack(const CfmRowsPackArgs& a, hipStream_t st);
int cfm_rows_emit(float* out, const float* x, const int* prompt_len, const int* gen_len, int B, int C, int T, int Tg_max, hipStream_t st);

int groupnorm1_mish(float* y, const float* x, const float* gamma, const float* beta, const int* row_len, int B, int T, int C,
                    float eps, float* stats , hipStream_t st);
int gather_tail_rows(float* dst, int ld_dst, const float* src, int ld_src, int cols, int N, int T, int t0, hipStream_t st);
int cfm_init_state(float* x, const float* z, const int* prompt_len, int B, int C, int T, hipStream_t st);

}
```

index-tts_amd/csrc/s2mel_ops.hip:

```cpp
#include "device_util.h"
#include "prof.h"
#include "s2mel_ops.h"

namespace idxtts {

__global__ __launch_bounds__(256) void rotary_qk_kernel(float* qkv, int M, int H, int seq_len, const float* rope) {
  const int pairs = 2 * H * 32;
  const size_t idx = (size_t)blockIdx.x * 256 + threadIdx.x;
  if (idx >= (size_t)M * pairs) return;
  const int m = (int)(idx / pairs), r = (int)(idx - (size_t)m * pairs);
  const int i = r & 31;
  const int t = m % seq_len;
  float2* ptr = reinterpret_cast<float2*>(qkv + (size_t)m * 3 * H * 64) + r;
  const float2 cs = reinterpret_cast<const float2*>(rope)[(size_t)t * 32 + i];
  const float2 v = *ptr;
  *ptr = float2{v.x * cs.x - v.y * cs.y, v.y * cs.x + v.x * cs.y};
}

int rotary_qk(float* qkv, int M, int H, int seq_len, const float* rope, hipStream_t st) {
  IDX_CHECK(qkv && rope && seq_len > 0, "rotary args");
  const size_t n = (size_t)M * 2 * H * 32;
  static const int cat = prof_register("rotary_qk_kernel");
  ProfScope prof(cat, st, 0.0, 16.0 * n);
  hipLaunchKernelGGL(rotary_qk_kernel, dim3((unsigned)cdiv64(n, 256)), dim3(256), 0, st, qkv, M, H, seq_len, rope);
  IDX_LAUNCH_CHECK();
  return 0;
}

__global__ __launch_bounds__(256) void silu_kernel(float* y, const float* x, size_t n) {
  const size_t i = (size_t)blockIdx.x * 256 + threadIdx.x;
  if (i < n) { const float v = x[i]; y[i] = v / (1.0f + expf(-v)); }
}

int silu_rows(float* y, const float* x, size_t n, hipStream_t st) {
  if (!n) return 0;
  hipLaunchKernelGGL(silu_kernel, dim3((unsigned)cdiv64(n, 256)), dim3(256), 0, st, y, x, n);
  IDX_LAUNCH_CHECK();
  return 0;
}

__global__ __launch_bounds__(256) void cfm_pack_kernel(const CfmPackArgs p) {
  const int n = blockIdx.y, b = n % p.B;
  const bool is_cond = n < p.B;
  const int t0 = blockIdx.x * 64;
  const int W = p.x_only ? p.C : 2 * p.C + p.D + p.S;
  const int Tp = p.prompt_len[b];
  for (int e = threadIdx.x; e < 64 * W; e += 256) {
    const int tt = e / W, c = e - tt * W;
    const int t = t0 + tt;
    if (t >= p.T) break;
    float v;
    if (c < p.C) v = p.x[((size_t)b * p.C + c) * p.T + t];
    else if (c < 2 * p.C) v = (is_cond && t < Tp) ? p.prompt[((size_t)b * p.C + (c - p.C)) * p.Tp_max + t] : 0.0f;
    else if (c < 2 * p.C + p.D) v = is_cond ? p.cond[((size_t)b * p.T + t) * p.D + (c - 2 * p.C)] : p.cond_null[c - 2 * p.C];
    else v = is_cond ? p.style[(size_t)b * p.S + (c - 2 * p.C - p.D)] : 0.0f;
    p.x_in[((size_t)n * p.T + t) * p.ld + c] = v;
  }
}

int cfm_pack(const CfmPackArgs& a, hipStream_t st) {
  const double bytes = 4.0 * 2 * a.B * (double)a.T * (a.x_only ? a.C : 2 * a.C + a.D + a.S) * 2;
  static const int cat = prof_register("cfm_pack_kernel");
  ProfScope prof(cat, st, 0.0, bytes);
  hipLaunchKernelGGL(cfm_pack_kernel, dim3(cdiv(a.T, 64), 2 * a.B), dim3(256), 0, st, a);
  IDX_LAUNCH_CHECK();
  return 0;
}

__global__ __launch_bounds__(256) void cfm_euler_kernel(const CfmEulerArgs p) {
  const size_t idx = (size_t)blockIdx.x * 256 + threadIdx.x;
  const size_t total = (size_t)p.B * p.C * p.T;
  if (idx >= total) return;
  const int t = (int)(idx % p.T);
  const int c = (int)((idx / p.T) % p.C);
  const int b = (int)(idx / ((size_t)p.T * p.C));
  if (t < p.prompt_len[b] || t < p.v_t0) { p.x[idx] = 0.0f; return; }
  const int vT = p.v_T > 0 ? p.v_T : p.T, tv = t - p.v_t0;
  const float vc = p.v[((size_t)b * vT + tv) * p.ldv + c];
  const float vn = p.v_null ? p.v_null[((size_t)b * vT + tv) * p.ldv + c] : p.v[((size_t)(p.B + b) * vT + tv) * p.ldv + c];
  const float dphi = (1.0f + p.cfg_rate) * vc - p.cfg_rate * vn;
  p.x[idx] = p.x[idx] + p.dt * dphi;
}

int cfm_euler(const CfmEulerArgs& a, hipStream_t st) {
  const size_t total = (size_t)a.B * a.C * a.T;
  static const int cat = prof_register("cfm_euler_kernel");
  ProfScope prof(cat, st, 0.0, 16.0 * total);
  hipLaunchKernelGGL(cfm_euler_kernel, dim3((unsigned)cdiv64(total, 256)), dim3(256), 0, st, a);
  IDX_LAUNCH_CHECK();
  return 0;
}

__global__ __launch_bounds__(256) void gather_tail_rows_kernel(float* dst, int ld_dst, const float* src, int ld_src, int cols, int T, int t0, int Tn) {
  const int j = blockIdx.x, n = blockIdx.y;
  const float* s = src + ((size_t)n * T + t0 + j) * ld_src;
  float* d = dst + ((size_t)n * Tn + j) * ld_dst;
  if (((cols | ld_dst | ld_src) & 3) == 0) {
    for (int e = threadIdx.x; e < cols / 4; e += 256) reinterpret_cast<f32x4*>(d)[e] = reinterpret_cast<const f32x4*>(s)[e];
  } else {
    for (int e = threadIdx.x; e < cols; e += 256) d[e] = s[e];
  }
}

int gather_tail_rows(float* dst, int ld_dst, const float* src, int ld_src, int cols, int N, int T, int t0, hipStream_t st) {
  IDX_CHECK(dst && src && t0 >= 0 && t0 < T && cols > 0, "gather_tail_rows args");
  const int Tn = T - t0;
  static const int cat = prof_register("gather_tail_rows_kernel");
  ProfScope prof(cat, st, 0.0, 8.0 * N * (double)Tn * cols);
  hipLaunchKernelGGL(gather_tail_rows_kernel, dim3(Tn, N), dim3(256), 0, st, dst, ld_dst, src, ld_src, cols, T, t0, Tn);
  IDX_LAUNCH_CHECK();
  return 0;
}

__global__ __launch_bounds__(256) void cfm_init_state_kernel(float* x, const float* z, const int* prompt_len, int B, int C, int T) {
  const size_t idx = (size_t)blockIdx.x * 256 + threadIdx.x;
  if (idx >= (size_t)B * C * T) return;
  const int t = (int)(idx % T), b = (int)(idx / ((size_t)T * C));
  x[idx] = t < prompt_len[b] ? 0.0f : z[idx];
}

int cfm_init_state(float* x, const float* z, const int* prompt_len, int B, int C, int T, hipStream_t st) {
  const size_t total = (size_t)B * C * T;
  hipLaunchKernelGGL(cfm_init_state_kernel, dim3((unsigned)cdiv64(total, 256)), dim3(256), 0, st, x, z, prompt_len, B, C, T);
  IDX_LAUNCH_CHECK();
  return 0;
}

__global__ __launch_bounds__(256) void cfm_rows_pack_kernel(const CfmRowsPackArgs p) {
  const int b = blockIdx.y, t0 = blockIdx.x * 64;
  const int Tp = p.prompt_len[b], Tg = p.gen_len[b];
  const int nt = min(64, p.T - t0);
  const int W = p.Dc / 4;
  const f32x4* pc = reinterpret_cast<const f32x4*>(p.pcond[b]);
  const f32x4* gen = reinterpret_cast<const f32x4*>(p.gen + (size_t)b * p.Tg_max * p.Dc);
  f32x4* mu = reinterpret_cast<f32x4*>(p.mu + ((size_t)b * p.T + t0) * p.Dc);
  for (int e = threadIdx.x; e < nt * W; e += 256) {
    const int tt = e / W, c = e - tt * W, t = t0 + tt;
    f32x4 v = {0.0f, 0.0f, 0.0f, 0.0f};
    if (t < Tp) v = pc[(size_t)t * W + c];
    else if (t < Tp + Tg) v = gen[(size_t)(t - Tp) * W + c];
    mu[(size_t)tt * W + c] = v;
  }
  if (t0 >= p.Tp_max) return;
  const int np = min(64, p.Tp_max - t0);
  const float* ref = p.ref_mel[b];
  for (int e = threadIdx.x; e < p.C * np; e += 256) {
    const int c = e / np, t = t0 + (e - c * np);
    p.prompt[((size_t)b * p.C + c) * p.Tp_max + t] = t < Tp ? ref[(size_t)c * Tp + t] : 0.0f;
  }
}

int cfm_rows_pack(const CfmRowsPackArgs& a, hipStream_t st) {
  IDX_CHECK(a.mu && a.prompt && a.pcond && a.ref_mel && a.gen && a.prompt_len && a.gen_len, "cfm_rows_pack args");
  IDX_CHECK(a.B > 0 && a.T > 0 && a.Dc > 0 && a.Dc % 4 == 0 && a.Tp_max > 0 && a.Tp_max <= a.T, "cfm_rows_pack shape");
  static const int cat = prof_register("cfm_rows_pack_kernel");
  ProfScope prof(cat, st, 0.0, 8.0 * a.B * ((double)a.T * a.Dc + (double)a.C * a.Tp_max));
  hipLaunchKernelGGL(cfm_rows_pack_kernel, dim3(cdiv(a.T, 64), a.B), dim3(256), 0, st, a);
  IDX_LAUNCH_CHECK();
  return 0;
}

__global__ __launch_bounds__(256) void cfm_rows_emit_kernel(float* out, const float* x, const int* prompt_len, const int* gen_len, int B,
                                                            int C, int T, int Tg_max) {
  const size_t idx = (size_t)blockIdx.x * 256 + threadIdx.x;
  if (idx >= (size_t)B * C * Tg_max) return;
  const int j = (int)(idx % Tg_max);
  const size_t bc = idx / Tg_max;
  const int b = (int)(bc / C);
  out[idx] = j < gen_len[b] ? x[bc * T + prompt_len[b] + j] : 0.0f;
}

int cfm_rows_emit(float* out, const float* x, const int* prompt_len, const int* gen_len, int B, int C, int T, int Tg_max, hipStream_t st) {
  IDX_CHECK(out && x && prompt_len && gen_len && B > 0 && C > 0 && Tg_max > 0 && Tg_max <= T, "cfm_rows_emit args");
  const size_t total = (size_t)B * C * Tg_max;
  static const int cat = prof_register("cfm_rows_emit_kernel");
  ProfScope prof(cat, st, 0.0, 8.0 * total);
  hipLaunchKernelGGL(cfm_rows_emit_kernel, dim3((unsigned)cdiv64(total, 256)), dim3(256), 0, st, out, x, prompt_len, gen_len, B, C, T, Tg_max);
  IDX_LAUNCH_CHECK();
  return 0;
}

__global__ __launch_bounds__(1024) void gn_stats_kernel(const float* x, const int* row_len, int T, int C, float* stats) {
  __shared__ float red[16];
  __shared__ float bc;
  const int b = blockIdx.x, tid = threadIdx.x;
  const size_t n = (size_t)row_len[b] * C;
  const float* xb = x + (size_t)b * T * C;
  float s = 0.f;
  for (size_t i = tid; i < n; i += 1024) s += xb[i];
  s = wave_sum(s);
  if ((tid & 63) == 0) red[tid >> 6] = s;
  __syncthreads();
  if (tid == 0) { float a = 0.f; for (int i = 0; i < 16; ++i) a += red[i]; bc = n ? a / (float)n : 0.f; }
  __syncthreads();
  const float mean = bc;
  float ss = 0.f;
  for (size_t i = tid; i < n; i += 1024) { const float c = xb[i] - mean; ss += c * c; }
  ss = wave_sum(ss);
  __syncthreads();
  if ((tid & 63) == 0) red[tid >> 6] = ss;
  __syncthreads();
  if (tid == 0) { float a = 0.f; for (int i = 0; i < 16; ++i) a += red[i]; stats[2 * b] = mean; stats[2 * b + 1] = n ? a / (float)n : 0.f; }
}

__global__ __launch_bounds__(256) void gn_apply_mish_kernel(float* y, const float* x, const float* gamma, const float* beta,
                                                            const int* row_len, const float* stats, int T, int C, float eps) {
  const int m = blockIdx.x;
  const int b = m / T, t = m - b * T;
  const bool valid = t < row_len[b];
  const float mean = stats[2 * b], rstd = rsqrtf(stats[2 * b + 1] + eps);
  for (int c = threadIdx.x; c < C; c += 256) {
    float o = 0.0f;
    if (valid) {
      const float v = (x[(size_t)m * C + c] - mean) * rstd * gamma[c] + beta[c];
      const float sp = v > 20.0f ? v : log1pf(expf(v));
      o = v * tanhf(sp);
    }
    y[(size_t)m * C + c] = o;
  }
}

int groupnorm1_mish(float* y, const float* x, const float* gamma, const float* beta, const int* row_len, int B, int T, int C,
                    float eps, float* stats, hipStream_t st) {
  static const int cat = prof_register("gn_stats_kernel + gn_apply_mish_kernel");
  ProfScope prof(cat, st, 0.0, 12.0 * B * (double)T * C);
  hipLaunchKernelGGL(gn_stats_kernel, dim3(B), dim3(1024), 0, st, x, row_len, T, C, stats);
  hipLaunchKernelGGL(gn_apply_mish_kernel, dim3(B * T), dim3(256), 0, st, y, x, gamma, beta, row_len, stats, T, C, eps);
  IDX_LAUNCH_CHECK();
  return 0;
}

}
```

Baseline: 190.1.

## Pack conv weight planes chunk-major and emit bf16 input planes from cfm_pack

Conv weights with multiple taps are repacked so each 16-channel chunk holds all taps together. In interior waves the GEMM can then step the A offset by a constant dilation stride instead of recomputing per-tap row offsets, and only edge waves fall back to per-tap address computation. Separately, cfm_pack and gather_tail_rows can write split hi/lo bf16 planes directly for the merge and skip-linear GEMMs. This removes the separate split_planes pass and the fp32 round trip for those inputs. The cost is extra plane buffers, a host-side weight reorder at load time, and a new consistency check tying weight packing to the tap count.

Result: no change. 191.1, median of 6 (+0.5%).

```diff
diff --git a/index-tts_amd/csrc/gemm.h b/index-tts_amd/csrc/gemm.h
--- a/index-tts_amd/csrc/gemm.h
+++ b/index-tts_amd/csrc/gemm.h
@@ -13,6 +13,7 @@
   const void* tiles16 = nullptr;
   const void* planes16 = nullptr;
   bool mf16 = false;
+  int plane_taps = 1;
 };
 
 static inline size_t linear_packed_floats(int N, int K) { return (size_t)cdiv(N, 32) * cdiv(K, 16) * 512; }
diff --git a/index-tts_amd/csrc/gemm_bf16x3_v2.hip b/index-tts_amd/csrc/gemm_bf16x3_v2.hip
--- a/index-tts_amd/csrc/gemm_bf16x3_v2.hip
+++ b/index-tts_amd/csrc/gemm_bf16x3_v2.hip
@@ -100,11 +100,13 @@
     const int t = conv_src_row(arow.t + tap * p.dil - p.pad_left, arow.n, p.pad_mode);
     return a_m < p.M && t >= 0 ? (arow.base + t) * 32 + dunit * 16 : (int)0x80000000;
   };
+  const bool edge_lane = TAPS && !(a_m < p.M && arow.t - p.pad_left >= 0 && arow.t - p.pad_left + (p.taps - 1) * p.dil < arow.n);
+  const bool edge_wave = TAPS && __builtin_amdgcn_ballot_w64(edge_lane) != 0;
+  const int tap_step = TAPS && !edge_wave ? p.dil * 32 : 0;
   V2_STAMP(0); V2_RSTAMP(4);
   const int ns = q.nstages;
   const int sA = q.a_rows * 32, sB = q.npad * 32;
-  const int cpt = TAPS ? (p.kc >> 4) : ns;
-  int ist = 0, soA = 0, soB = 0, ich = 0, itap = 0, wslot = 0, rslot = 0;
+  int ist = 0, soA = 0, soB = 0, itap = 0, wslot = 0, rslot = 0;
   if (TAPS) voffA = tap_voff(0);
   char* const lds_w = smv2 + wave * 1024;
   auto issue_piece = [&](int pi) {
@@ -120,9 +122,12 @@
     ++ist;
     wslot = wslot + 1 == NSTAGE ? 0 : wslot + 1;
     soB += sB;
-    soA += sA;
     if (TAPS) {
-      if (++ich == cpt) { ich = 0; soA = 0; ++itap; voffA = tap_voff(itap); }
+      if (++itap == p.taps) { itap = 0; soA += sA - (p.taps - 1) * tap_step; }
+      else soA += tap_step;
+      if (edge_wave) voffA = tap_voff(itap);
+    } else {
+      soA += sA;
     }
   };
 
@@ -353,6 +358,7 @@
 
 int gemm_bf16x3_v2_forward(GemmKP p, const LinearWeights& w, const GemmArgs& a, hipStream_t stream, double flops, double bytes) {
   IDX_CHECK(w.K % 16 == 0 && (a.taps <= 1 || (w.K / a.taps) % 16 == 0), "v2 needs K % 16 == 0");
+  IDX_CHECK(std::max(1, a.taps) == w.plane_taps, "the weight planes are packed for another tap count (LinearOpts::taps)");
   const int xk = a.taps > 1 ? w.K / a.taps : w.K;
   const size_t plane = (size_t)(xk / 16) * a.M * 16 * sizeof(__bf16);
   void* scratch = nullptr;
diff --git a/index-tts_amd/csrc/model_util.h b/index-tts_amd/csrc/model_util.h
--- a/index-tts_amd/csrc/model_util.h
+++ b/index-tts_amd/csrc/model_util.h
@@ -26,6 +26,7 @@
   WeightLayout layout = W_NK;
   int Kpad = 0;
   bool split_bf16_below_256_rows = false;
+  int taps = 1;
 };
 int make_linear(DeviceArena& arena, const float* w, const float* bias, int N, int K, const LinearOpts& o, LinearWeights* out);
 int linear_from(std::map<std::string, HostTensor>& t, DeviceArena& arena, const std::string& prefix, int N, int K, bool bias, Wp16Policy wp16,
diff --git a/index-tts_amd/csrc/model_util.hip b/index-tts_amd/csrc/model_util.hip
--- a/index-tts_amd/csrc/model_util.hip
+++ b/index-tts_amd/csrc/model_util.hip
@@ -65,8 +65,21 @@
     return 0;
   };
   const bool planes = o.wp16 != WP16_NONE && linear_takes_planes(N, Kpad);
+  std::vector<float> by_chunk;
+  const float* const w_tap_major = w;
+  if (planes && o.taps > 1) {
+    IDX_CHECK(Kpad == K && K % o.taps == 0 && (K / o.taps) % 16 == 0, "conv weights: K / taps must be a multiple of 16");
+    const int kc = K / o.taps;
+    by_chunk.resize((size_t)N * K);
+    for (int n = 0; n < N; ++n)
+      for (int tap = 0; tap < o.taps; ++tap)
+        for (int c = 0; c < kc; ++c) by_chunk[(size_t)n * K + ((size_t)(c >> 4) * o.taps + tap) * 16 + (c & 15)] = w[(size_t)n * K + (size_t)tap * kc + c];
+    w = by_chunk.data();
+    out->plane_taps = o.taps;
+  }
   const bool tiles = o.wp16 != WP16_NONE && (o.split_bf16_below_256_rows || (o.wp16 != WP16_DMA_SHAPES && !planes));
   if (planes && pack16(linear_planes_bytes(N, Kpad), pack_linear_planes, &out->planes16)) return 1;
+  w = w_tap_major;
   if (tiles && pack16(linear_tiles_bytes(N, Kpad), pack_linear_tiles, &out->tiles16)) return 1;
   if (bias && up(arena, std::vector<float>(bias, bias + N), &out->bias)) return 1;
   return 0;
diff --git a/index-tts_amd/csrc/s2mel.hip b/index-tts_amd/csrc/s2mel.hip
--- a/index-tts_amd/csrc/s2mel.hip
+++ b/index-tts_amd/csrc/s2mel.hip
@@ -59,6 +59,11 @@
   const std::string e = "cfm.estimator";
   auto lin_from = [&](const std::string& key, int N, int K, bool bias, LinearWeights* out) { return linear_from(t, arena, key, N, K, bias, WP16_ALWAYS_MF16, out); };
   auto mk_lin = [&](const float* w, const float* bias, int N, int K, LinearWeights* out) { return make_linear(arena, w, bias, N, K, {WP16_ALWAYS_MF16}, out); };
+  auto mk_conv = [&](const float* w, const float* bias, int N, int K, int taps, LinearWeights* out) {
+    LinearOpts o{WP16_ALWAYS_MF16};
+    o.taps = taps;
+    return make_linear(arena, w, bias, N, K, o, out);
+  };
   blocks.resize(depth);
   std::vector<float> mod_w, mod_b;
   auto append_mod = [&](const std::string& name) -> int {
@@ -127,7 +132,7 @@
       HostTensor *iw = nullptr, *ib = nullptr;
       if (need(t, p + ".weight", {2 * Wh, Wh, k}, &iw) || need(t, p + ".bias", {2 * Wh}, &ib)) return 1;
       const std::vector<float> rows = conv_to_rows(iw->data, 2 * Wh, Wh, k);
-      if (mk_lin(pair_pack(rows.data(), rows.data() + (size_t)Wh * k * Wh, Wh, k * Wh).data(), nullptr, 2 * Wh, k * Wh, &W.in_gate)) return 1;
+      if (mk_conv(pair_pack(rows.data(), rows.data() + (size_t)Wh * k * Wh, Wh, k * Wh).data(), nullptr, 2 * Wh, k * Wh, k, &W.in_gate)) return 1;
       const float* cwl = cw->data.data() + (size_t)l * 2 * Wh * Wh;
       const std::vector<float> cwp = pair_pack(cwl, cwl + (size_t)Wh * Wh, Wh, Wh);
       cw_perm.insert(cw_perm.end(), cwp.begin(), cwp.end());
@@ -159,7 +164,7 @@
     HostTensor *w = nullptr, *b = nullptr, *g = nullptr, *bb = nullptr;
     const std::string p = "length_regulator.model." + std::to_string(3 * n);
     if (need(t, p + ".weight", {LC, LC, 3}, &w) || need(t, p + ".bias", {LC}, &b)) return 1;
-    if (mk_lin(conv_to_rows(w->data, LC, LC, 3).data(), b->data.data(), LC, 3 * LC, &lr_conv[n])) return 1;
+    if (mk_conv(conv_to_rows(w->data, LC, LC, 3).data(), b->data.data(), LC, 3 * LC, 3, &lr_conv[n])) return 1;
     const std::string q = "length_regulator.model." + std::to_string(3 * n + 1);
     if (need(t, q + ".weight", {LC}, &g) || need(t, q + ".bias", {LC}, &bb)) return 1;
     if (up(arena, g->data, &lr_gn_g[n]) || up(arena, bb->data, &lr_gn_b[n])) return 1;
@@ -222,6 +227,7 @@
   const int* lens = nullptr;
   bool planes = false;
   bool planes_wn = false;
+  bool planes_xin = false, planes_xcol = false;
 
   Src hn_in() const { return in(w->hn, w->hn_p, planes); }                  Dst hn_out() const { return instead(w->hn, w->hn_p, planes); }
   Src att_in() const { return in(w->att, w->att_p, planes); }               Dst att_out() const { return instead(w->att, w->att_p, planes); }
@@ -230,6 +236,7 @@
   Src skip_in(int i) const { return in(w->skips[i], w->skips_p[i], planes); }   Dst skip_out(int i) const { return beside(w->skips[i], w->skips_p[i], planes); }
   Src xres_in() const { return in(w->xres, w->xres_p, planes_wn); }         Dst xres_out() const { return beside(w->xres, w->xres_p, planes_wn); }
   Src wnx_in() const { return in(w->wn_x, w->wnx_p, planes_wn); }           Dst wnx_out() const { return beside(w->wn_x, w->wnx_p, planes_wn); }
+  Src xin_in() const { return in(w->x_in, w->xin_p, planes_xin); }
   Src h_in(const float* h) const { return in(h, w->h_p, planes); }          Dst h_out(float* h, bool reread) const { return beside(h, w->h_p, planes && reread); }
 
  private:
@@ -251,7 +258,20 @@
   for (const LinearWeights* lw : {&m.skiplin_b, &m.conv1, &m.res_proj, &wn0.res}) r.planes_wn = r.planes_wn && gemm_uses_planes(*lw, pr);
   pr.taps = m.cfg.wn_kernel; pr.seq_len = seq;
   r.planes_wn = r.planes_wn && gemm_uses_planes(wn0.in_gate, pr);
+  const auto& c = m.cfg;
+  const bool packable = c.in_channels % 16 == 0 && c.hidden_dim % 4 == 0 && c.style_dim % 4 == 0;
+  pr.taps = 1; pr.seq_len = 0;
+  r.planes_xin = !within && packable && gemm_uses_planes(m.merge, pr);
+  r.planes_xcol = packable && gemm_uses_planes(m.skiplin_b, pr);
   return r;
+}
+
+struct EvalRows { RowSet all, tail; };
+static EvalRows eval_rows(const S2MelModel& m, const CfmBuffers& w, int N2, int T) {
+  EvalRows e;
+  e.all = row_set(m, w, N2, T, w.lens2, nullptr);
+  e.tail = w.tail_t0 > 0 ? row_set(m, w, N2, T - w.tail_t0, w.lens2t, &e.all) : e.all;
+  return e;
 }
 
 static int ada_norm(const S2MelModel& m, const float* x, const float* g, const float* mod, const RowSet& r, hipStream_t st) {
@@ -302,7 +322,7 @@
   }
   if (attention(m, all, qkv_planes, q0, post.seq, post.att_out(), st)) return 1;
   if (lag_event) IDX_HIP(hipEventRecord(lag_event, st));
-  if (res != h && gather_tail_rows(res, D, h, D, D, all.nseq, T, q0, st)) return 1;
+  if (res != h && gather_tail_rows(res, nullptr, D, h, D, D, all.nseq, T, q0, st)) return 1;
   if (gemm(B.wo, post.att_in(), D, w.hmid, D, post.rows, st, ACT_NONE, res, D)) return 1;
   if (ada_norm(m, w.hmid, B.ffn_g, mods + (size_t)(2 * i + 1) * 2 * D, post, st)) return 1;
   if (gemm(B.w13, post.hn_in(), D, post.ff_out(), m.ffn, post.rows, st, ACT_SWIGLU)) return 1;
@@ -315,10 +335,10 @@
   const int Win = 2 * C + D + c.style_dim;
   const float* mods = w.mods + (size_t)step * (2 * depth + 1) * 2 * D;
   const int t0 = w.tail_t0;
-  const RowSet all = row_set(m, w, N2, T, w.lens2, nullptr);
-  const RowSet tail = t0 > 0 ? row_set(m, w, N2, T - t0, w.lens2t, &all) : all;
+  const EvalRows er = eval_rows(m, w, N2, T);
+  const RowSet &all = er.all, &tail = er.tail;
   if (lag_event && depth < 2) IDX_HIP(hipEventRecord(lag_event, st));
-  if (gemm(m.merge, w.x_in, Win, w.ha, D, all.rows, st)) return 1;
+  if (gemm(m.merge, all.xin_in(), Win, w.ha, D, all.rows, st)) return 1;
   float* h = w.ha;
   int pushed = 0;
   for (int i = 0; i < depth; ++i) {
@@ -337,11 +357,14 @@
     h = out.f;
   }
   const int Mt = tail.rows, Tt = tail.seq;
-  const float* xin_t = w.x_in;
+  Src xin_t(w.x_in);
   int ld_xin = Win;
   if (t0 > 0) {
-    if (gather_tail_rows(w.qkv, C, w.x_in, Win, C, N2, T, t0, st)) return 1;
-    xin_t = w.qkv; ld_xin = C;
+    const Dst xc = tail.planes_xcol ? Dst(nullptr, w.xcol_p) : Dst(w.qkv);
+    if (gather_tail_rows(xc.f, xc.p, C, w.x_in, Win, C, N2, T, t0, st)) return 1;
+    xin_t = Src(w.qkv, xc.p); ld_xin = C;
+  } else if (tail.planes_xcol) {
+    xin_t = Src(nullptr, w.xcol_p); ld_xin = C;
   }
   if (ada_norm(m, h, m.final_g, mods + (size_t)(2 * depth) * 2 * D, tail, st)) return 1;
   if (gemm(m.skiplin_a, tail.hn_in(), D, w.hmid, D, Mt, st)) return 1;
@@ -490,9 +513,13 @@
   return gemm(m.wn_cond, w.t2, Wh, w.wnb, m.cfg.wn_layers * 2 * Wh, n_steps, st);
 }
 
-static CfmPackArgs pack_args(const S2MelModel& m, const CfmBuffers& w, const float* prompt, const float* style, int B, int T, int Tp_max) {
+static CfmPackArgs pack_args(const S2MelModel& m, const CfmBuffers& w, const float* prompt, const float* style, int B, int T, int Tp_max, int N2) {
   const auto& c = m.cfg;
   CfmPackArgs pk;
+  const EvalRows er = eval_rows(m, w, N2, T);
+  if (er.all.planes_xin) pk.x_in_p = w.xin_p;
+  if (er.tail.planes_xcol && w.tail_t0 == 0) pk.xcol_p = w.xcol_p;
+  pk.seq_p = N2; pk.t0 = w.tail_t0;
   pk.x_in = w.x_in; pk.ld = 2 * c.in_channels + c.hidden_dim + c.style_dim; pk.x = w.xstate; pk.prompt = prompt; pk.prompt_len = w.plen;
   pk.cond = w.condp; pk.cond_null = m.cond_proj.bias; pk.style = style;
   pk.B = B; pk.T = T; pk.C = c.in_channels; pk.D = c.hidden_dim; pk.S = c.style_dim; pk.Tp_max = Tp_max;
@@ -509,7 +536,7 @@
   if (cfm_init_state(w.xstate, z, w.plen, B, C, T, st)) return 1;
   const bool two_streams = halves_on_two_streams(st);
   for (int s = 0; s < n_steps; ++s) {
-    CfmPackArgs pk = pack_args(*this, w, prompt, style, B, T, Tp_max);
+    CfmPackArgs pk = pack_args(*this, w, prompt, style, B, T, Tp_max, two_streams ? B : 2 * B);
     pk.x_only = s > 0;
     if (cfm_pack(pk, st)) return 1;
     if (dit_eval_halves(*this, w, B, T, s, two_streams, st)) return 1;
@@ -590,7 +617,7 @@
   if (step_constants(*this, w, t_emb, 1, st)) return 1;
   if (gemm(cond_proj, mu, cfg.content_dim, w.condp, cfg.hidden_dim, B * T, st)) return 1;
   IDX_HIP(hipMemcpyAsync(w.xstate, x, (size_t)B * C * T * sizeof(float), hipMemcpyDeviceToDevice, st));
-  if (cfm_pack(pack_args(*this, w, prompt, style, B, T, Tp_max), st)) return 1;
+  if (cfm_pack(pack_args(*this, w, prompt, style, B, T, Tp_max, B), st)) return 1;
   {
     CfmBuffers v0 = half_view(cfg, ffn, w, 0, B, T);
     if (dit_eval(*this, v0, B, T, 0, st, nullptr)) return 1;
diff --git a/index-tts_amd/csrc/s2mel_buffers.h b/index-tts_amd/csrc/s2mel_buffers.h
--- a/index-tts_amd/csrc/s2mel_buffers.h
+++ b/index-tts_amd/csrc/s2mel_buffers.h
@@ -11,6 +11,7 @@
   float *x_in, *ha, *hb, *hmid, *hn, *qkv, *att, *ff, *xres, *wn_x, *wn_acts, *wn_out, *vout, *condp, *xstate;
   void *hn_p, *att_p, *ff_p, *acts_p;
   void *h_p, *wnx_p, *xres_p;
+  void *xin_p, *xcol_p;
   std::vector<void*> skips_p;
   std::vector<float*> skips;
   float *t1, *t1s, *mods, *fmod, *t2, *wnb, *tmp_steps;
@@ -39,6 +40,7 @@
   f(b.qkv, 3 * D, R, H); f(b.att, D, R, H); f(b.ff, ffn, R, H); f(b.xres, D, R, H);
   f(b.hn_p, std::max(D, Wh), P, H); f(b.att_p, D, P, H); f(b.ff_p, ffn, P, H); f(b.acts_p, Wh, P, H);
   f(b.h_p, D, P, H); f(b.wnx_p, Wh, P, H); f(b.xres_p, D, P, H);
+  f(b.xin_p, 2 * C + D + c.style_dim, P, H); f(b.xcol_p, C, P, H);
   f(b.wn_x, Wh, R, H); f(b.wn_acts, Wh, R, H); f(b.wn_out, Wh, R, H); f(b.vout, C, R, H);
   f(b.condp, D, R, CFM_SHARED);
   f(b.xstate, C, R, CFM_SHARED);
diff --git a/index-tts_amd/csrc/s2mel_ops.h b/index-tts_amd/csrc/s2mel_ops.h
--- a/index-tts_amd/csrc/s2mel_ops.h
+++ b/index-tts_amd/csrc/s2mel_ops.h
@@ -16,6 +16,9 @@
   const float* style;
   int B, T, C, D, S, Tp_max;
   int x_only = 0;
+  void* x_in_p = nullptr;
+  void* xcol_p = nullptr;
+  int seq_p = 0, t0 = 0;
 };
 int cfm_pack(const CfmPackArgs& a, hipStream_t st);
 
@@ -45,7 +48,7 @@
 
 int groupnorm1_mish(float* y, const float* x, const float* gamma, const float* beta, const int* row_len, int B, int T, int C,
                     float eps, float* stats , hipStream_t st);
-int gather_tail_rows(float* dst, int ld_dst, const float* src, int ld_src, int cols, int N, int T, int t0, hipStream_t st);
+int gather_tail_rows(float* dst, void* dst_planes, int ld_dst, const float* src, int ld_src, int cols, int N, int T, int t0, hipStream_t st);
 int cfm_init_state(float* x, const float* z, const int* prompt_len, int B, int C, int T, hipStream_t st);
 
 }
diff --git a/index-tts_amd/csrc/s2mel_ops.hip b/index-tts_amd/csrc/s2mel_ops.hip
--- a/index-tts_amd/csrc/s2mel_ops.hip
+++ b/index-tts_amd/csrc/s2mel_ops.hip
@@ -58,11 +58,57 @@
   }
 }
 
+__global__ __launch_bounds__(256) void cfm_pack_planes_kernel(const CfmPackArgs p) {
+  const int n = blockIdx.y, b = n % p.B;
+  const bool is_cond = n < p.B;
+  const int t = blockIdx.x * 64 + (threadIdx.x >> 2);
+  if (t >= p.T) return;
+  const int W = p.x_only ? p.C : 2 * p.C + p.D + p.S;
+  const int Tp = p.prompt_len[b];
+  const int blk = n / p.seq_p, nn = n - blk * p.seq_p, Tt = p.T - p.t0;
+  const int rows = p.seq_p * p.T, rows_t = p.seq_p * Tt;
+  __bf16* const xin_hi = p.x_in_p ? static_cast<__bf16*>(p.x_in_p) + (size_t)blk * 2 * rows * p.ld : nullptr;
+  __bf16* const xin_lo = xin_hi + (size_t)rows * p.ld;
+  __bf16* const xc_hi = p.xcol_p ? static_cast<__bf16*>(p.xcol_p) + (size_t)blk * 2 * rows * p.C : nullptr;
+  __bf16* const xc_lo = xc_hi + (size_t)rows_t * p.C;
+  for (int c = (threadIdx.x & 3) * 4; c < W; c += 16) {
+    f32x4 v;
+#pragma unroll
+    for (int i = 0; i < 4; ++i) {
+      const int cc = c + i;
+      if (cc < p.C) v[i] = p.x[((size_t)b * p.C + cc) * p.T + t];
+      else if (cc < 2 * p.C) v[i] = (is_cond && t < Tp) ? p.prompt[((size_t)b * p.C + (cc - p.C)) * p.Tp_max + t] : 0.0f;
+      else if (cc < 2 * p.C + p.D) v[i] = is_cond ? p.cond[((size_t)b * p.T + t) * p.D + (cc - 2 * p.C)] : p.cond_null[cc - 2 * p.C];
+      else v[i] = is_cond ? p.style[(size_t)b * p.S + (cc - 2 * p.C - p.D)] : 0.0f;
+    }
+    idx_bf16x4 h, l;
+    split_bf16_x4(v, h, l);
+    if (xin_hi) {
+      const size_t o = plane_index(nn * p.T + t, c, rows);
+      *reinterpret_cast<idx_bf16x4*>(xin_hi + o) = h;
+      *reinterpret_cast<idx_bf16x4*>(xin_lo + o) = l;
+    }
+    if (xc_hi && c < p.C && t >= p.t0) {
+      const size_t o = plane_index(nn * Tt + t - p.t0, c, rows_t);
+      *reinterpret_cast<idx_bf16x4*>(xc_hi + o) = h;
+      *reinterpret_cast<idx_bf16x4*>(xc_lo + o) = l;
+    }
+    if (!xin_hi || (c < p.C && !xc_hi)) *reinterpret_cast<f32x4*>(p.x_in + ((size_t)n * p.T + t) * p.ld + c) = v;
+  }
+}
+
 int cfm_pack(const CfmPackArgs& a, hipStream_t st) {
   const double bytes = 4.0 * 2 * a.B * (double)a.T * (a.x_only ? a.C : 2 * a.C + a.D + a.S) * 2;
   static const int cat = prof_register("cfm_pack_kernel");
   ProfScope prof(cat, st, 0.0, bytes);
-  hipLaunchKernelGGL(cfm_pack_kernel, dim3(cdiv(a.T, 64), 2 * a.B), dim3(256), 0, st, a);
+  if (a.x_in_p || a.xcol_p) {
+    IDX_CHECK(((a.C | a.D | a.S | a.ld) & 3) == 0 && (a.seq_p == a.B || a.seq_p == 2 * a.B) && a.t0 >= 0 && a.t0 < a.T, "cfm_pack planes args");
+    IDX_CHECK(!a.x_in_p || ((a.C | a.ld) & 15) == 0, "x_in planes need C and ld to be multiples of 16");
+    IDX_CHECK(!a.xcol_p || (a.C & 15) == 0, "x-column planes need C to be a multiple of 16");
+    hipLaunchKernelGGL(cfm_pack_planes_kernel, dim3(cdiv(a.T, 64), 2 * a.B), dim3(256), 0, st, a);
+  } else {
+    hipLaunchKernelGGL(cfm_pack_kernel, dim3(cdiv(a.T, 64), 2 * a.B), dim3(256), 0, st, a);
+  }
   IDX_LAUNCH_CHECK();
   return 0;
 }
@@ -102,11 +148,31 @@
   }
 }
 
-int gather_tail_rows(float* dst, int ld_dst, const float* src, int ld_src, int cols, int N, int T, int t0, hipStream_t st) {
-  IDX_CHECK(dst && src && t0 >= 0 && t0 < T && cols > 0, "gather_tail_rows args");
+__global__ __launch_bounds__(256) void gather_tail_planes_kernel(__bf16* hi, const float* src, int ld_src, int cols, int T, int t0, int Tn, int rows) {
+  const int j = blockIdx.x * 64 + (threadIdx.x >> 2), n = blockIdx.y;
+  if (j >= Tn) return;
+  const float* s = src + ((size_t)n * T + t0 + j) * ld_src;
+  __bf16* const lo = hi + (size_t)rows * cols;
+  for (int c = (threadIdx.x & 3) * 4; c < cols; c += 16) {
+    idx_bf16x4 h, l;
+    split_bf16_x4(*reinterpret_cast<const f32x4*>(s + c), h, l);
+    const size_t o = plane_index(n * Tn + j, c, rows);
+    *reinterpret_cast<idx_bf16x4*>(hi + o) = h;
+    *reinterpret_cast<idx_bf16x4*>(lo + o) = l;
+  }
+}
+
+int gather_tail_rows(float* dst, void* dst_planes, int ld_dst, const float* src, int ld_src, int cols, int N, int T, int t0, hipStream_t st) {
+  IDX_CHECK((dst || dst_planes) && src && t0 >= 0 && t0 < T && cols > 0, "gather_tail_rows args");
   const int Tn = T - t0;
   static const int cat = prof_register("gather_tail_rows_kernel");
   ProfScope prof(cat, st, 0.0, 8.0 * N * (double)Tn * cols);
+  if (dst_planes) {
+    IDX_CHECK(!dst && cols % 16 == 0 && (ld_src & 3) == 0 && (reinterpret_cast<uintptr_t>(src) & 15) == 0, "gather_tail_rows: planes need cols % 16 == 0 and 16-byte rows");
+    hipLaunchKernelGGL(gather_tail_planes_kernel, dim3(cdiv(Tn, 64), N), dim3(256), 0, st, static_cast<__bf16*>(dst_planes), src, ld_src, cols, T, t0, Tn, N * Tn);
+    IDX_LAUNCH_CHECK();
+    return 0;
+  }
   hipLaunchKernelGGL(gather_tail_rows_kernel, dim3(Tn, N), dim3(256), 0, st, dst, ld_dst, src, ld_src, cols, T, t0, Tn);
   IDX_LAUNCH_CHECK();
   return 0;
```
